# LittlePey/TASeg

Measured on AMD Instinct MI355X. Metric: scans/sec (train fwd+bwd) at ~120k pts/scan, higher is better.
Workload: dtype f32

## Files before the change

### include/taseg_hip.h

```cpp
#ifndef TASEG_HIP_H_
#define TASEG_HIP_H_

#include <stddef.h>
#include <stdint.h>

#ifdef __cplusplus
extern "C" {
#endif

#define TS_OK 0
#define TS_ERR_INVALID_ARGUMENT (-1)
#define TS_ERR_WORKSPACE_TOO_SMALL (-2)
#define TS_ERR_LAUNCH_FAILED (-3)
#define TS_ERR_UNSUPPORTED (-4)

typedef void *ts_stream_t;

const char *ts_version(void);
const char *ts_last_error(void);

enum {
  TS_OPT_GATHER_POSITIONS = 0,
  TS_OPT_WGRAD_WGS = 1,
  TS_OPT_EVAL_TAIL_SEPARATE = 2,
// ... 371 lines not shown
                      const void *labels, int32_t label_bytes, int64_t n_lab, const int64_t *num_points,
                      const int64_t *num_points_ms, int64_t *hist, int32_t *pred, int64_t pred_cap, int32_t *flags,
                      ts_stream_t stream);
int ts_eval_votes(const void *logits, int32_t half, int32_t C, int64_t n_vox, const int64_t *counts, const int32_t *scene_flags,
                  int32_t n_scenes, const int64_t *inv, const int32_t *rows, const int64_t *kept, int64_t n_pts,
                  const int64_t *num_points, const int64_t *num_points_ms, void *label, int32_t label_bytes, float *sums,
                  float *top3, int64_t cap, int64_t *n_out, int32_t *flags, ts_stream_t stream);
int ts_eval_confusion_rows(const void *logits, int32_t half, int32_t C, int64_t n_vox, const int64_t *counts,
                           const int32_t *scene_flags, int32_t n_scenes, const int64_t *grows, int64_t n_pts, const void *labels,
                           int32_t label_bytes, const int64_t *num_points, int64_t *hist, int32_t *pred, int64_t pred_cap,
                           int64_t *m_out, int32_t *flags, ts_stream_t stream);
int ts_eval_votes_rows(const void *logits, int32_t half, int32_t C, int64_t n_vox, const int64_t *counts, const int32_t *scene_flags,
                       int32_t n_scenes, const int64_t *grows, int64_t n_pts, const int64_t *num_points, void *label,
                       int32_t label_bytes, float *sums, float *top3, int64_t cap, int64_t *n_out, int32_t *flags,
                       ts_stream_t stream);
int ts_cat_cols(const void *a, int64_t a_bytes, const void *b, int64_t b_bytes, int64_t rows, void *dst, ts_stream_t stream);
int ts_copy_cols(const void *src, int64_t src_pitch, int64_t offset, int64_t width, int64_t rows, void *dst, int64_t dst_pitch,
                 ts_stream_t stream);
int ts_conv_block_forward(const void *feat, int64_t n_feat_rows, int32_t c_in, const float *kernel, int32_t K,
                          const int32_t *nbmaps, const int32_t *nboffs, int64_t n_pairs, int32_t gather_col,
                          const int32_t *pos, int64_t n_out, int32_t c_out, const void *residual, const float *bn_weight,
                          const float *bn_bias, float *running_mean, float *running_var, int64_t *num_batches_tracked,
                          float eps, float momentum, int32_t relu, int32_t half, void *comm, double *pack, void *conv_out,
                          float *mean, float *invstd, void *out, uint8_t *mask, void *w16, const TsConvBlockOpts *opts,
                          void *ws, size_t ws_bytes, ts_stream_t stream);
int ts_conv_block_eval(const void *feat, int64_t n_feat_rows, int32_t c_in, const float *kernel, int32_t K,
                       const int32_t *nbmaps, const int32_t *nboffs, int64_t n_pairs, int32_t gather_col, const int32_t *pos,
                       int64_t n_out, int32_t c_out, const void *residual, const float *bn_weight, const float *bn_bias,
                       const float *mean, const float *invstd, int32_t relu, int32_t half, void *out, void *w16,
                       const TsConvBlockOpts *opts, void *ws, size_t ws_bytes, ts_stream_t stream);
int ts_conv_block_backward(const void *grad_out, const uint8_t *mask, const void *conv_out, const float *mean,
                           const float *invstd, const float *bn_weight, const double *total_dev, void *comm, double *sums,
                           int64_t n_out, int32_t c_out, int32_t half, const void *feat, int64_t n_feat_rows, int32_t c_in,
                           const void *weights, int32_t K, const int32_t *nbmaps, const int32_t *nboffs, int64_t n_pairs,
                           int32_t dgrad_gather_col, const int32_t *pos_dgrad, int64_t n_dgrad_rows, int32_t wgrad_col_a,
                           void *grad_feat, void *grad_residual, float *grad_kernel, float *grad_bn_weight,
                           float *grad_bn_bias, const TsConvBlockOpts *opts, void *ws, size_t ws_bytes, ts_stream_t stream);

void ts_prof_enable(int32_t on);
int ts_prof_reserve(int64_t n_events);
int64_t ts_prof_collect(double *records, int64_t capacity);
int ts_prof_empty_bracket_us(int32_t reps, ts_stream_t stream, double *out_us);

void ts_set_conv_impl(int32_t impl);

int ts_lovasz_errors(const float *probas, const int64_t *labels, int64_t ignore, int64_t n_points, int32_t n_classes,
                     float *errors, ts_stream_t stream);
size_t ts_lovasz_workspace_bytes(int64_t n_points, int32_t n_classes);
int ts_lovasz_grad(const float *errors_sorted, const int64_t *perm, const int64_t *labels, int64_t ignore, int64_t n_points,
                   int32_t n_classes, float *loss, float *grad_probas, int32_t class_major, void *ws, size_t ws_bytes,
                   ts_stream_t stream);

int ts_softmax_ce_forward(const float *logits, const int64_t *labels, int64_t ignore, int64_t n_points, int32_t n_classes,
                          float *probas, float *errors, double *partials, ts_stream_t stream);
int ts_ce_lovasz_finish(const double *partials, int64_t n_points, int32_t n_classes, float smoothing, float w_ce, float w_lov,
                        const float *lovasz, float *out4, ts_stream_t stream);
int ts_ce_lovasz_backward(const float *probas, const int64_t *labels, int64_t ignore, const float *grad_probas,
                          const float *out4, const float *grad_out, int64_t n_points, int32_t n_classes, float smoothing,
                          float w_ce, float w_lov, float *grad_logits, ts_stream_t stream);

typedef struct TsPlaneJob {
  const float *w;
  void *planes;
  int32_t K, c_in, c_out;
} TsPlaneJob;
int ts_conv_split_planes(const float *w, int32_t K, int32_t c_in, int32_t c_out, void *planes, ts_stream_t stream);
int ts_conv_split_planes_batch(const TsPlaneJob *jobs, int32_t n_jobs, ts_stream_t stream);
void ts_conv_planes_hint(const float *w, const void *planes, int32_t K, int32_t c_in, int32_t c_out);
int ts_cast_weights_f16_batch(const TsPlaneJob *jobs, int32_t n_jobs, ts_stream_t stream);

int64_t ts_conv_class_rows(int64_t n);
int64_t ts_conv_class_rows2(int64_t n, int32_t groups);
size_t ts_conv_class_plan_workspace_bytes(int64_t n);
int ts_conv_class_plan(const int32_t *nbr, int64_t n, int32_t K, int32_t groups, int32_t *src, int32_t *tile_info,
                       int32_t *n_tiles, int32_t *pos, int32_t *rows, void *ws, size_t ws_bytes, ts_stream_t stream);
int ts_conv_class_plan_pairs(const int32_t *nbmaps, const int32_t *nboffs, int32_t K, int64_t n_pairs, int32_t *src,
                             int32_t *tile_info, int32_t *n_tiles, int32_t *rows, void *ws, size_t ws_bytes, ts_stream_t stream);
int ts_conv_nbr_transposed(const int32_t *pos_in, const int32_t *nbmaps, int32_t K, int64_t n_in, int32_t *nbr_t,
                           ts_stream_t stream);
int32_t ts_conv_class_supported(int32_t c_red, int32_t c_out);
int ts_conv_class_gemm(const float *feat, int32_t c_red, const float *kernel, int32_t K, int32_t groups, int32_t c_out,
                       const int32_t *src, int64_t m_pad, const int32_t *tile_info, const int32_t *n_tiles, int32_t wt,
                       int32_t mirror, const int32_t *rows, float *zp, ts_stream_t stream);
int32_t ts_conv_class_finish_pays(int64_t n, int32_t half);
int ts_conv_class_conv(const float *feat, int32_t c_red, const float *kernel, int32_t K, int32_t groups, int32_t c_out,
                       const int32_t *src, int64_t m_pad, const int32_t *tile_info, const int32_t *n_tiles, int32_t wt,
                       int32_t mirror, const int32_t *pos, int64_t n, const float *addend, float *zp, float *out,
                       ts_stream_t stream);
int ts_conv_class_gemm_f16(const void *feat, int32_t c_red, const void *w, int32_t K, int32_t groups, int32_t c_out,
                           const int32_t *src, int64_t m_pad, const int32_t *tile_info, const int32_t *n_tiles, int32_t wt,
                           int32_t mirror, const int32_t *rows, void *zp, ts_stream_t stream);
int ts_conv_class_conv_f16(const void *feat, int32_t c_red, const void *w, int32_t K, int32_t groups, int32_t c_out,
                           const int32_t *src, int64_t m_pad, const int32_t *tile_info, const int32_t *n_tiles, int32_t wt,
                           int32_t mirror, const int32_t *pos, int64_t n, const void *addend, void *zp, void *out,
                           ts_stream_t stream);

void ts_debug_phase_stamps(unsigned long long *stamps, int64_t capacity);


int ts_voxel_coords(const float *points, int64_t n, int32_t point_stride, float voxel_size,
                    const int32_t *batch_idx, int32_t n_batch, const int32_t *shift_in,
                    int32_t *mins_out, int32_t *out_coords, ts_stream_t stream);

int ts_segment_min3(const float *points, int64_t n, int32_t point_stride, const int64_t *seg, int32_t n_seg, float *out,
                    ts_stream_t stream);
int ts_stage_keep_flags(const float *points, int64_t n, int32_t point_stride, const uint8_t *pre_keep, const int32_t *scan_idx,
                        const int64_t *cls, const uint8_t *table, int32_t n_scans, int32_t table_cols, int32_t neg_col,
                        const int64_t *sample_of_scan, const float *lo, int32_t n_samples, uint8_t *keep, int64_t *sample,
                        ts_stream_t stream);
int ts_stage_layout(const float *cur, const int64_t *cur_lab, const int64_t *cur_b, int64_t n_cur, const float *hist,
                    const int64_t *hist_lab, const int64_t *hist_b, const int64_t *idx, int64_t n_kept, int32_t f,
                    const int64_t *cur_start, const int64_t *kept_start, float *pts, int64_t *lab, int64_t *sample, int32_t *sample32,
                    uint8_t *is_cur, ts_stream_t stream);
int ts_stage_split_voxels(const int32_t *coords4, const int32_t *index, int64_t m, const int32_t *inverse,
                          const int64_t *row_sample, int64_t n, int32_t n_samples, int32_t *vox, int64_t *start, int32_t *offset,
                          int64_t *inverse_local, ts_stream_t stream);
#define TS_AUG_RECORD 8
int ts_stage_augment(const float *points, int64_t n, int32_t point_stride, const int32_t *sample_idx, const double *params,
                     int32_t n_samples, float *out, ts_stream_t stream);
#define TS_MIX_RECORD 24
#define TS_MIX_MAX_CLASSES 16
size_t ts_stage_mix_workspace_bytes(int64_t n_rows, int64_t n_blocks, int32_t n_jobs);
int ts_stage_mix(const float *points, int64_t n_rows, int32_t point_stride, const int64_t *labels, const uint8_t *keep,
                 const double *records, const int32_t *classes, int32_t n_jobs, int64_t n_blocks, float *out, int64_t *out_labels,
                 int32_t *out_job, int64_t capacity, int64_t *totals, void *ws, size_t ws_bytes, ts_stream_t stream);
#define TS_CLAMP_MAX_SAMPLES 64
size_t ts_stage_clamp_compact_workspace_bytes(int64_t n, int32_t n_samples);
int ts_stage_clamp_compact(const float *points, int64_t n, int32_t point_stride, const int64_t *labels, const int32_t *sample,
                           const float *lo, int32_t n_samples, float *out, int64_t *out_labels, int64_t *out_sample,
                           int32_t *out_sample32, int64_t *counts, void *ws, size_t ws_bytes, ts_stream_t stream);
#define TS_STAGE_PAIR_MAX_SAMPLES 64
size_t ts_stage_layout_pair_workspace_bytes(int64_t n_hist, int32_t n_samples);
int ts_stage_layout_pair(const float *cur, int64_t n_cur, int32_t cur_stride, const int64_t *cur_labels, const int64_t *cur_start,
                         const float *hist, int64_t n_hist, const int64_t *hist_labels, const int32_t *scan_idx,
                         const int64_t *cls_a, const int64_t *cls_b, const uint8_t *table_a, const uint8_t *table_b,
                         int32_t n_scans, int32_t table_cols, int32_t neg_col, const int64_t *sample_of_scan, const float *lo,
                         int32_t n_samples, float *out_a, int64_t *out_labels_a, int64_t *out_sample_a, int32_t *out_sample32_a,
                         uint8_t *out_is_cur_a, float *out_b, int64_t *out_sample_b, int32_t *out_sample32_b, int64_t capacity,
                         int64_t *counts, void *ws, size_t ws_bytes, ts_stream_t stream);
#define TS_MOVING_STATS 9
#define TS_MOVING_RECORD 8
#define TS_MOVING_MAX_CANDIDATES 1024
size_t ts_stage_moving_workspace_bytes(int64_t n_rows, int32_t cap, int64_t cap_rows);
int ts_stage_moving_stats(const float *points, int64_t n_rows, int64_t n_cur, int32_t point_stride, const int64_t *labels,
                          const int32_t *cloud, const int32_t *delta, const int64_t *cand, const int32_t *cand_start,
                          int32_t n_clouds, int32_t cap, int64_t cap_rows, int32_t *counts, float *stats, int64_t *matched, void *ws,
                          size_t ws_bytes, ts_stream_t stream);
int ts_stage_moving_apply(float *points, int64_t n_rows, int64_t n_cur, int32_t point_stride, const int64_t *labels,
                          const int32_t *cloud, const int32_t *delta, const int64_t *rec_labels, const int32_t *rec_start,
                          int32_t n_clouds, const double *records, const int64_t *lut, int64_t *out_labels, ts_stream_t stream);
size_t ts_quantize_workspace_bytes(int64_t n);
int ts_sparse_quantize(const int32_t *coords, int64_t n, int32_t *out_index, int32_t *out_inverse,
                       int32_t *out_count, void *ws, size_t ws_bytes, ts_stream_t stream);
#define TS_CYL_FLAG_WORDS 3
#define TS_CYL_FLAG_NONFINITE 1
#define TS_CYL_FLAG_LABEL 2
#define TS_CYL_FLAG_RANGE 4
int ts_cylinder_cells(const float *points, int64_t n, int32_t point_stride, const int32_t *sample_idx, const double *space,
                      int32_t *cells, int64_t *point_coord, float *point_feature, int32_t *flags, ts_stream_t stream);
size_t ts_cylinder_voxels_workspace_bytes(int64_t n, int32_t n_samples);
int ts_cylinder_voxels(const int32_t *cells, const int64_t *labels, int64_t n, int32_t n_samples, int32_t num_classes,
                       int64_t ignore_label, int32_t *out_index, int64_t *out_inverse, int64_t *voxel_label, int32_t *counts,
                       int32_t *flags, void *ws, size_t ws_bytes, ts_stream_t stream);

int ts_fuse_scan(const float *points, int64_t n, const float *pose0, const float *pose,
                 float *out, ts_stream_t stream);
// ... 62 lines not shown
```

### taseg_amd/_lib.py

```python
import ctypes
import os
import threading

import torch

_HERE = os.path.dirname(os.path.abspath(__file__))
from .options import options as _options

LIB_PATH = _options.hip_lib or os.path.join(_HERE, "libtaseg_hip.so")

TS_OK = 0
_c = ctypes
_vp, _i64, _i32, _sz = _c.c_void_p, _c.c_int64, _c.c_int32, _c.c_size_t

SIGNATURES = {
    "ts_version": (_c.c_char_p, []),
    "ts_last_error": (_c.c_char_p, []),
    "ts_set_option": (_i32, [_i32, _i64]),
    "ts_get_option": (_i64, [_i32]),
    "ts_hash": (_i32, [_vp, _i64, _vp, _vp]),
    "ts_kernel_hash": (_i32, [_vp, _i64, _vp, _i32, _vp, _vp]),
    "ts_hash_query_workspace_bytes": (_sz, [_i64]),
    "ts_hash_query": (_i32, [_vp, _i64, _vp, _vp, _i64, _vp, _vp, _sz, _vp]),
    "ts_count": (_i32, [_vp, _i64, _vp, _i64, _vp]),
# ... 80 lines not shown
    "ts_conv3x3_rows_pack": (_i32, [_vp, _i32, _i32, _i64, _i64, _i64, _i64, _i32, _vp, _vp]),
    "ts_conv3x3_rows": (_i32, [_vp, _i32, _vp, _vp, _i32, _i32, _i32, _vp, _i32, _vp]),
    "ts_conv1x1c32_packed_bytes": (_sz, []),
    "ts_conv1x1c32_pack": (_i32, [_vp, _i64, _i64, _i32, _vp, _vp]),
    "ts_conv1x1c32_rows": (_i32, [_vp, _vp, _vp, _i64, _i32, _c.c_float, _vp, _vp]),
    "ts_conv1x1c32_wgrad": (_i32, [_vp, _vp, _i32, _i32, _i32, _vp, _i64, _i64, _vp, _vp, _sz, _vp]),
    "ts_conv3x3_wgrad_workspace_bytes": (_sz, [_i32, _i32]),
    "ts_conv3x3_wgrad": (_i32, [_vp, _i32, _vp, _i32, _i32, _i32, _i32, _vp, _i64, _i64, _i64, _i64, _vp, _vp, _sz, _vp]),
    "ts_conv3x3c32_wgrad_workspace_bytes": (_sz, []),
    "ts_conv3x3c32_wgrad": (_i32, [_vp, _vp, _i32, _i32, _i32, _i32, _vp, _i64, _i64, _i64, _i64, _vp, _vp, _sz, _vp]),
    "ts_cast_weights_f16": (_i32, [_vp, _i32, _i32, _i32, _vp, _vp, _vp]),
    "ts_conv_pair_gemm_f16": (_i32, [_vp, _i64, _i32, _vp, _i32, _vp, _vp, _i64, _i32, _vp, _i32, _vp]),
    "ts_conv_pair_gemm_f16_nat": (_i32, [_vp, _i64, _i32, _vp, _i32, _vp, _vp, _i64, _i32, _vp, _i32, _vp]),
    "ts_conv_gather_sum_f16": (_i32, [_vp, _i32, _vp, _i32, _i64, _i64, _vp, _vp]),
    "ts_conv_wgrad_f16": (_i32, [_vp, _i32, _vp, _i32, _vp, _vp, _i32, _i32, _i64, _vp, _vp]),
    "ts_bn_act_train_forward_f16": (_i32, [_vp, _vp, _vp, _vp, _vp, _vp, _vp, _i64, _i32, _c.c_float, _c.c_float, _i32,
                                           _vp, _vp, _vp, _vp, _vp, _sz, _vp]),
    "ts_bn_act_train_backward_f16": (_i32, [_vp, _vp, _vp, _vp, _vp, _vp, _i64, _i32, _vp, _vp, _vp, _vp, _vp, _sz, _vp]),
    "ts_sgd_grad_stats": (_i32, [_vp, _i64, _vp, _vp, _vp]),
    "ts_sgd_decide": (_i32, [_vp, _vp, _vp, _c.c_float, _c.c_float, _c.c_float, _i32, _i32, _vp]),
    "ts_sgd_apply": (_i32, [_vp, _vp, _vp, _i64, _vp, _c.c_float, _c.c_float, _c.c_float, _i32, _vp]),
    "ts_sgd_apply_segments": (_i32, [_vp, _vp, _vp, _i64, _vp, _vp, _i32, _vp, _i64, _vp, _vp, _i32, _c.c_float, _c.c_float,
                                     _c.c_float, _i32, _i32, _vp]),
    "ts_bn_sync_stats_f16": (_i32, [_vp, _i64, _i32, _vp, _vp, _sz, _vp]),
    "ts_bn_act_forward_f16": (_i32, [_vp, _vp, _vp, _vp, _vp, _vp, _i64, _i32, _i32, _vp, _vp, _vp]),
    "ts_bn_sync_backward_reduce_f16": (_i32, [_vp, _vp, _vp, _vp, _vp, _i64, _i32, _vp, _vp, _vp, _vp, _sz, _vp]),
    "ts_bn_act_backward_f16": (_i32, [_vp, _vp, _vp, _vp, _vp, _vp, _vp, _vp, _c.c_double, _i64, _i32, _vp, _vp, _vp, _sz,
                                      _vp]),
    "ts_rccl_load": (_i32, [_c.c_char_p]),
    "ts_rccl_unique_id": (_i32, [_vp]),
    "ts_rccl_comm_init": (_i32, [_vp, _i32, _i32, _c.POINTER(_vp)]),
    "ts_rccl_comm_destroy": (_i32, [_vp]),
    "ts_rccl_allreduce_f64": (_i32, [_vp, _vp, _i64, _vp]),
    "ts_bn_sync_forward": (_i32, [_vp, _vp, _vp, _vp, _vp, _vp, _vp, _vp, _i64, _i32, _c.c_float, _c.c_float, _i32, _i32, _vp,
                                  _vp, _vp, _vp, _vp, _vp, _sz, _vp]),
    "ts_bn_sync_backward": (_i32, [_vp, _vp, _vp, _vp, _vp, _vp, _vp, _vp, _i64, _i32, _i32, _vp, _vp, _vp, _vp, _vp, _vp,
                                   _sz, _vp]),
    "ts_conv_block_workspace_bytes": (_sz, [_i64, _i64, _i32, _i32, _i32, _i32]),
    "ts_conv_block_wgrad_ws_bytes": (_sz, [_i64, _i64, _i32, _i32, _i32, _i32]),
    "ts_stream_join": (_i32, [_vp, _vp]),
    "ts_conv_block_wgrad_side": (_i32, [_vp, _i64, _i32, _i32, _vp, _vp, _i64, _i32, _i64, _i32, _i32, _vp, _i32, _vp, _sz, _i32, _vp]),
    "ts_set_device": (_i32, [_i32]),
    "ts_scene_counts": (_i32, [_vp, _i64, _i64, _vp, _i64, _i64, _vp, _i64, _i64, _i32, _vp, _vp, _vp]),
    "ts_unvoxelise": (_i32, [_vp, _i32, _i32, _vp, _i32, _vp, _i64, _vp, _i64, _vp, _vp, _vp, _vp]),
    "ts_eval_rows_workspace_bytes": (_sz, [_i64, _i32]),
    "ts_eval_rows": (_i32, [_vp, _vp, _i64, _vp, _i64, _i32, _vp, _vp, _vp, _sz, _vp]),
    "ts_eval_confusion": (_i32, [_vp, _i32, _i32, _i64, _vp, _vp, _i32, _vp, _vp, _vp, _i64, _vp, _i32, _i64, _vp, _vp, _vp, _vp, _i64,
                                 _vp, _vp]),
    "ts_eval_votes": (_i32, [_vp, _i32, _i32, _i64, _vp, _vp, _i32, _vp, _vp, _vp, _i64, _vp, _vp, _vp, _i32, _vp, _vp, _i64, _vp, _vp,
                             _vp]),
    "ts_eval_confusion_rows": (_i32, [_vp, _i32, _i32, _i64, _vp, _vp, _i32, _vp, _i64, _vp, _i32, _vp, _vp, _vp, _i64, _vp, _vp, _vp]),
    "ts_eval_votes_rows": (_i32, [_vp, _i32, _i32, _i64, _vp, _vp, _i32, _vp, _i64, _vp, _vp, _i32, _vp, _vp, _i64, _vp, _vp, _vp]),
    "ts_cat_cols": (_i32, [_vp, _i64, _vp, _i64, _i64, _vp, _vp]),
    "ts_copy_cols": (_i32, [_vp, _i64, _i64, _i64, _i64, _vp, _i64, _vp]),
    "ts_conv_block_forward": (_i32, [_vp, _i64, _i32, _vp, _i32, _vp, _vp, _i64, _i32, _vp, _i64, _i32, _vp, _vp, _vp, _vp,
                                     _vp, _vp, _c.c_float, _c.c_float, _i32, _i32, _vp, _vp, _vp, _vp, _vp, _vp, _vp, _vp,
                                     _vp, _vp, _sz, _vp]),
    "ts_conv_block_eval": (_i32, [_vp, _i64, _i32, _vp, _i32, _vp, _vp, _i64, _i32, _vp, _i64, _i32, _vp, _vp, _vp, _vp, _vp, _i32,
                                  _i32, _vp, _vp, _vp, _vp, _sz, _vp]),
    "ts_conv_block_backward": (_i32, [_vp, _vp, _vp, _vp, _vp, _vp, _vp, _vp, _vp, _i64, _i32, _i32, _vp, _i64, _i32, _vp,
                                      _i32, _vp, _vp, _i64, _i32, _vp, _i64, _i32, _vp, _vp, _vp, _vp, _vp, _vp, _vp, _sz,
                                      _vp]),
    "ts_prof_enable": (None, [_i32]),
    "ts_prof_reserve": (_i32, [_i64]),
    "ts_prof_collect": (_i64, [_vp, _i64]),
    "ts_prof_empty_bracket_us": (_i32, [_i32, _vp, _vp]),
    "ts_set_conv_impl": (None, [_i32]),
    "ts_softmax_ce_forward": (_i32, [_vp, _vp, _i64, _i64, _i32, _vp, _vp, _vp, _vp]),
    "ts_ce_lovasz_finish": (_i32, [_vp, _i64, _i32, _c.c_float, _c.c_float, _c.c_float, _vp, _vp, _vp]),
    "ts_ce_lovasz_backward": (_i32, [_vp, _vp, _i64, _vp, _vp, _vp, _i64, _i32, _c.c_float, _c.c_float, _c.c_float, _vp, _vp]),
    "ts_lovasz_errors": (_i32, [_vp, _vp, _i64, _i64, _i32, _vp, _vp]),
    "ts_lovasz_workspace_bytes": (_sz, [_i64, _i32]),
    "ts_lovasz_grad": (_i32, [_vp, _vp, _vp, _i64, _i64, _i32, _vp, _vp, _i32, _vp, _sz, _vp]),
    "ts_conv_split_planes": (_i32, [_vp, _i32, _i32, _i32, _vp, _vp]),
    "ts_conv_split_planes_batch": (_i32, [_vp, _i32, _vp]),
    "ts_cast_weights_f16_batch": (_i32, [_vp, _i32, _vp]),
    "ts_conv_class_rows": (_i64, [_i64]),
    "ts_conv_class_rows2": (_i64, [_i64, _i32]),
    "ts_conv_class_plan_workspace_bytes": (_sz, [_i64]),
    "ts_conv_class_plan": (_i32, [_vp, _i64, _i32, _i32, _vp, _vp, _vp, _vp, _vp, _vp, _sz, _vp]),
    "ts_conv_class_plan_pairs": (_i32, [_vp, _vp, _i32, _i64, _vp, _vp, _vp, _vp, _vp, _sz, _vp]),
    "ts_conv_nbr_transposed": (_i32, [_vp, _vp, _i32, _i64, _vp, _vp]),
    "ts_conv_class_supported": (_i32, [_i32, _i32]),
    "ts_conv_class_gemm": (_i32, [_vp, _i32, _vp, _i32, _i32, _i32, _vp, _i64, _vp, _vp, _i32, _i32, _vp, _vp, _vp]),
    "ts_conv_class_gemm_f16": (_i32, [_vp, _i32, _vp, _i32, _i32, _i32, _vp, _i64, _vp, _vp, _i32, _i32, _vp, _vp, _vp]),
    "ts_conv_class_finish_pays": (_i32, [_i64, _i32]),
    "ts_conv_class_conv": (_i32, [_vp, _i32, _vp, _i32, _i32, _i32, _vp, _i64, _vp, _vp, _i32, _i32, _vp, _i64, _vp, _vp, _vp, _vp]),
    "ts_conv_class_conv_f16": (_i32, [_vp, _i32, _vp, _i32, _i32, _i32, _vp, _i64, _vp, _vp, _i32, _i32, _vp, _i64, _vp, _vp, _vp, _vp]),
    "ts_conv_planes_hint": (None, [_vp, _vp, _i32, _i32, _i32]),
    "ts_debug_phase_stamps": (None, [_vp, _i64]),
    "ts_fuse_scan": (_i32, [_vp, _i64, _vp, _vp, _vp, _vp]),
    "ts_fuse_scans": (_i32, [_vp, _vp, _i64, _vp, _vp, _i32, _vp, _vp]),
    "ts_fuse_scans_batch": (_i32, [_vp, _vp, _i64, _vp, _vp, _i32, _vp, _vp]),
    "ts_fuse_sweeps": (_i32, [_vp, _vp, _i64, _vp, _i32, _vp, _vp, _vp]),
    "ts_project_fov": (_i32, [_vp, _i64, _vp, _i32, _i32, _i32, _i32, _c.c_float, _vp, _vp, _vp]),
    "ts_project_cam": (_i32, [_vp, _i64, _vp, _i32, _i32, _i32, _c.c_float, _vp, _vp, _vp]),
    "ts_tiaf_image_stack": (_i32, [_vp, _vp, _vp, _vp, _vp, _i32, _vp, _i32, _i32, _i64, _i64, _vp, _vp, _vp]),
    "ts_tiaf_fov_cloud_workspace_bytes": (_sz, [_i64, _i32]),
    "ts_tiaf_fov_cloud": (_i32, [_vp, _i64, _vp, _i64, _vp, _i32, _vp, _vp, _i32, _i32, _i32, _vp, _vp, _vp, _i64, _vp, _vp, _sz, _vp]),
    "ts_nusc_fov_cloud_workspace_bytes": (_sz, [_i64, _i32]),
    "ts_nusc_fov_cloud": (_i32, [_vp, _vp, _vp, _i64, _vp, _i64, _vp, _i32, _vp, _vp, _i32, _vp, _vp, _vp, _vp, _i64, _vp, _vp, _sz, _vp]),
    "ts_segment_min3": (_i32, [_vp, _i64, _i32, _vp, _i32, _vp, _vp]),
    "ts_stage_keep_flags": (_i32, [_vp, _i64, _i32, _vp, _vp, _vp, _vp, _i32, _i32, _i32, _vp, _vp, _i32, _vp, _vp, _vp]),
    "ts_stage_augment": (_i32, [_vp, _i64, _i32, _vp, _vp, _i32, _vp, _vp]),
    "ts_stage_mix_workspace_bytes": (_sz, [_i64, _i64, _i32]),
    "ts_stage_mix": (_i32, [_vp, _i64, _i32, _vp, _vp, _vp, _vp, _i32, _i64, _vp, _vp, _vp, _i64, _vp, _vp, _sz, _vp]),
    "ts_stage_clamp_compact_workspace_bytes": (_sz, [_i64, _i32]),
    "ts_stage_clamp_compact": (_i32, [_vp, _i64, _i32, _vp, _vp, _vp, _i32, _vp, _vp, _vp, _vp, _vp, _vp, _sz, _vp]),
    "ts_stage_layout_pair_workspace_bytes": (_sz, [_i64, _i32]),
    "ts_stage_layout_pair": (_i32, [_vp, _i64, _i32, _vp, _vp, _vp, _i64, _vp, _vp, _vp, _vp, _vp, _vp, _i32, _i32, _i32, _vp, _vp,
                                    _i32, _vp, _vp, _vp, _vp, _vp, _vp, _vp, _vp, _i64, _vp, _vp, _sz, _vp]),
    "ts_stage_moving_workspace_bytes": (_sz, [_i64, _i32, _i64]),
    "ts_stage_moving_stats": (_i32, [_vp, _i64, _i64, _i32, _vp, _vp, _vp, _vp, _vp, _i32, _i32, _i64, _vp, _vp, _vp, _vp, _sz, _vp]),
    "ts_stage_moving_apply": (_i32, [_vp, _i64, _i64, _i32, _vp, _vp, _vp, _vp, _vp, _i32, _vp, _vp, _vp, _vp]),
    "ts_stage_layout": (_i32, [_vp, _vp, _vp, _i64, _vp, _vp, _vp, _vp, _i64, _i32, _vp, _vp, _vp, _vp, _vp, _vp, _vp, _vp]),
    "ts_stage_split_voxels": (_i32, [_vp, _vp, _i64, _vp, _vp, _i64, _i32, _vp, _vp, _vp, _vp, _vp]),
    "ts_quantize_workspace_bytes": (_sz, [_i64]),
    "ts_sparse_quantize": (_i32, [_vp, _i64, _vp, _vp, _vp, _vp, _sz, _vp]),
    "ts_voxel_coords": (_i32, [_vp, _i64, _i32, _c.c_float, _vp, _i32, _vp, _vp, _vp, _vp]),
    "ts_cylinder_cells": (_i32, [_vp, _i64, _i32, _vp, _c.POINTER(_c.c_double), _vp, _vp, _vp, _vp, _vp]),
    "ts_cylinder_voxels_workspace_bytes": (_sz, [_i64, _i32]),
    "ts_cylinder_voxels": (_i32, [_vp, _vp, _i64, _i32, _i32, _i64, _vp, _vp, _vp, _vp, _vp, _vp, _sz, _vp]),
}



SGD_TILE = 4096


class TsClassPlan(_c.Structure):
    _fields_ = [("src", _vp), ("tile_info", _vp), ("n_tiles", _vp), ("pos", _vp), ("rows", _vp), ("n", _i64), ("m_pad", _i64),
                ("z_rows", _i64), ("K", _i32), ("groups", _i32), ("mirror", _i32), ("map_id", _vp)]


class TsConvBlockOpts(_c.Structure):
    _fields_ = [("fwd_plan", _c.POINTER(TsClassPlan)), ("dgrad_plan", _c.POINTER(TsClassPlan)), ("planes", _vp),
                ("w16_current", _i32), ("addend", _vp), ("wgrad_stream", _vp), ("wgrad_ws", _vp), ("wgrad_ws_bytes", _sz),
                ("wgrad_slot", _i32), ("wgrad_deferred", _i32), ("natural", _i32)]


_lib = None
_lock = threading.Lock()


class BackendError(RuntimeError):
    """A libtaseg_hip entry point returned a TS_ERR_* code."""


def load():
    global _lib
    if _lib is not None:
        return _lib
    with _lock:
        if _lib is None:
            if not os.path.exists(LIB_PATH):
                raise ImportError(
                    f"{LIB_PATH} is missing: build it with `python -m taseg_amd.csrc.build` "
                    "(or __graft_entry__.build()).  taseg_amd has no CPU fallback.")
            lib = ctypes.CDLL(LIB_PATH)
            for name, (res, args) in SIGNATURES.items():
                fn = getattr(lib, name)
                fn.restype = res
                fn.argtypes = args
            push_options(lib)
            _lib = lib
    return _lib
# ... 55 lines not shown
```

### taseg_amd/backend.py

```python
import torch

from . import _lib as L
from ._lib import BackendError, check
from .options import options

__all__ = [
    "hash_cuda", "kernel_hash_cuda", "hash_query_cuda", "count_cuda",
    "voxelize_forward_cuda", "voxelize_backward_cuda",
    "devoxelize_forward_cuda", "devoxelize_backward_cuda", "devox_order", "devoxelize_backward_runs", "devox_csr",
    "devoxelize_backward_csr",
    "convolution_forward_cuda", "convolution_backward_cuda",
    "downsample", "unique_i64", "build_kmap", "trilinear_map", "conv_nbr", "conv_wgrad", "conv_class_plan", "conv_class_gemm", "conv_class_gemm_f16", "conv_class_conv", "conv_class_conv_f16", "class_finish_pays",
    "fuse_scan", "fuse_scans", "fuse_sweeps", "project_fov", "voxel_coords", "sparse_quantize", "set_conv_impl", "image_gather_forward", "image_gather_backward", "image_gather_rows_forward", "image_gather_rows_backward", "avgpool3s2_rows_forward", "avgpool3s2_rows_backward", "conv3x3c32_pack", "conv3x3c32_rows", "conv3x3c32_wgrad", "conv3x3_rows_takes", "conv3x3_rows_pack", "conv3x3_rows", "conv3x3_wgrad", "conv1x1c32_pack", "conv1x1c32_rows", "conv1x1c32_wgrad", "shuffle_cat_rows_takes", "shuffle_cat_rows_forward", "shuffle_cat_rows_backward",
    "eval_confusion", "eval_votes", "eval_confusion_rows", "eval_votes_rows",
    "voxelize_max_forward", "voxelize_max_backward", "sigmoid3_gate_forward", "sigmoid3_gate_backward",
    "point_groups", "voxelize_mean_piece_rows", "voxelize_mean_forward", "voxelize_mean_backward", "point_tail_forward",
]


def _f32(t, name):
    if t.dtype != torch.float32:
        raise TypeError(f"{name} must be float32 (got {t.dtype}); the HIP path computes in f32")
    return t.contiguous()

# ... 894 lines not shown
            raise ValueError("conv3x3_rows: bias length")
    y = torch.empty((t, int(out_channels), h, w), dtype=x.dtype, device=x.device, memory_format=torch.channels_last)
    L.check(lib.ts_conv3x3_rows(L.ptr(x), c, L.ptr(packed), L.ptr(bias), t, h, w, L.ptr(y), int(out_channels), L.stream()),
            "ts_conv3x3_rows")
    return y


def conv1x1c32_pack(weight, mode):
    L.require_device(weight)
    if weight.dtype != torch.float16 or tuple(weight.shape) != (32, 32, 1, 1):
        raise ValueError(f"conv1x1c32_pack: a float16 [32, 32, 1, 1] weight, got {weight.dtype} {tuple(weight.shape)}")
    lib = L.load()
    packed = torch.empty(lib.ts_conv1x1c32_packed_bytes(), dtype=torch.uint8, device=weight.device)
    L.check(lib.ts_conv1x1c32_pack(L.ptr(weight), weight.stride(0), weight.stride(1), int(mode), L.ptr(packed), L.stream()), "ts_conv1x1c32_pack")
    return packed


def conv1x1c32_rows(x, packed, bias, slope=None):
    L.require_device(x, packed, bias)
    x = _channels_last_rows(x, "conv1x1c32_rows")
    t, c, h, w = x.shape
    if c != 32 or x.dtype != torch.float16:
        raise ValueError(f"conv1x1c32_rows: float16 with 32 channels, got {x.dtype} with {c}")
    if bias is not None:
        bias = _f32(bias, "bias")
    y = torch.empty_like(x, memory_format=torch.channels_last)
    L.check(L.load().ts_conv1x1c32_rows(L.ptr(x), L.ptr(packed), L.ptr(bias), t * h * w, int(slope is not None), float(slope or 0.0), L.ptr(y),
                                        L.stream()), "ts_conv1x1c32_rows")
    return y


def conv1x1c32_wgrad(x, g, like_weight):
    L.require_device(x, g)
    x, g = _channels_last_rows(x, "conv1x1c32_wgrad(x)"), _channels_last_rows(g, "conv1x1c32_wgrad(g)")
    if x.shape != g.shape or x.shape[1] != 32 or x.dtype != torch.float16 or g.dtype != torch.float16 or tuple(like_weight.shape) != (32, 32, 1, 1):
        raise ValueError("conv1x1c32_wgrad: two float16 [T, 32, H, W] stacks of one shape and a [32, 32, 1, 1] weight")
    t, _, h, w = x.shape
    gw = torch.empty_like(like_weight, dtype=torch.float16)
    gb = torch.empty(32, dtype=torch.float32, device=x.device)
    lib = L.load()
    ws = L.workspace(lib.ts_conv3x3c32_wgrad_workspace_bytes(), x.device)
    L.check(lib.ts_conv1x1c32_wgrad(L.ptr(x), L.ptr(g), t, h, w, L.ptr(gw), gw.stride(0), gw.stride(1), L.ptr(gb), L.ptr(ws), ws.numel(), L.stream()),
            "ts_conv1x1c32_wgrad")
    return gw, gb


def conv3x3_wgrad(x, grad_y, like_weight, want_bias=True):
    L.require_device(x, grad_y)
    x, grad_y = _channels_last_rows(x, "conv3x3_wgrad(x)"), _channels_last_rows(grad_y, "conv3x3_wgrad(grad_y)")
    t, ci, h, w = x.shape
    co = grad_y.shape[1]
    lib = L.load()
    need = lib.ts_conv3x3_wgrad_workspace_bytes(ci, co)
    if (x.dtype != torch.float16 or grad_y.dtype != torch.float16 or tuple(grad_y.shape) != (t, co, h, w) or need == 0
            or tuple(like_weight.shape) != (co, ci, 3, 3)):
        raise ValueError(f"conv3x3_wgrad: float16 stacks {tuple(x.shape)} / {tuple(grad_y.shape)} and a weight like {tuple(like_weight.shape)}")
    gw = torch.empty_like(like_weight, dtype=torch.float16)
    gb = torch.empty(co, dtype=torch.float32, device=x.device) if want_bias else None
    s = gw.stride()
    ws = L.workspace(need, x.device)
    L.check(lib.ts_conv3x3_wgrad(L.ptr(x), ci, L.ptr(grad_y), co, t, h, w, L.ptr(gw), s[0], s[1], s[2], s[3], L.ptr(gb), L.ptr(ws), ws.numel(),
                                 L.stream()), "ts_conv3x3_wgrad")
    return gw, gb


def conv3x3c32_wgrad(x, grad_y, like_weight, dilation, want_bias=False):
    L.require_device(x, grad_y)
    x, grad_y = _channels_last_rows(x, "conv3x3c32_wgrad(x)"), _channels_last_rows(grad_y, "conv3x3c32_wgrad(grad_y)")
    if x.shape != grad_y.shape or x.shape[1] != 32 or x.dtype != torch.float16 or grad_y.dtype != torch.float16:
        raise ValueError("conv3x3c32_wgrad: two float16 [T, 32, H, W] stacks of one shape")
    t, _, h, w = x.shape
    gw = torch.empty_like(like_weight, dtype=torch.float16)
    gb = torch.empty(32, dtype=torch.float32, device=x.device) if want_bias else None
    s = gw.stride()
    lib = L.load()
    ws = L.workspace(lib.ts_conv3x3c32_wgrad_workspace_bytes(), x.device)
    L.check(lib.ts_conv3x3c32_wgrad(L.ptr(x), L.ptr(grad_y), t, h, w, int(dilation), L.ptr(gw), s[0], s[1], s[2], s[3], L.ptr(gb), L.ptr(ws),
                                    ws.numel(), L.stream()), "ts_conv3x3c32_wgrad")
    return (gw, gb) if want_bias else gw


def set_conv_impl(impl):
    global _conv_impl
    _conv_impl = int(impl)
    L.load().ts_set_conv_impl(int(impl))


def fuse_scan(points, pose0, pose):
    L.require_device(points, pose0, pose)
    points, pose0, pose = _f32(points, "points"), _f32(pose0, "pose0"), _f32(pose, "pose")
    assert points.ndim == 2 and points.shape[1] == 4 and pose0.shape == (4, 4) and pose.shape == (4, 4)
    out = torch.empty_like(points)
    L.check(L.load().ts_fuse_scan(L.ptr(points), points.shape[0], L.ptr(pose0), L.ptr(pose), L.ptr(out), L.stream()),
            "ts_fuse_scan")
    return out


def fuse_scans(points, scan_idx, pose0, poses):
    L.require_device(points, scan_idx, pose0, poses)
    points, pose0, poses = _f32(points, "points"), _f32(pose0, "pose0"), _f32(poses, "poses")
    scan_idx = _i32(scan_idx, "scan_idx")
    assert points.ndim == 2 and points.shape[1] == 4 and pose0.shape == (4, 4) and poses.shape[1:] == (4, 4)
    out = torch.empty_like(points)
    L.check(L.load().ts_fuse_scans(L.ptr(points), L.ptr(scan_idx), points.shape[0], L.ptr(pose0), L.ptr(poses),
                                   poses.shape[0], L.ptr(out), L.stream()), "ts_fuse_scans")
    return out


def fuse_scans_batch(points, scan_idx, pose0s, poses):
    L.require_device(points, scan_idx, pose0s, poses)
    points, pose0s, poses = _f32(points, "points"), _f32(pose0s, "pose0s"), _f32(poses, "poses")
    scan_idx = _i32(scan_idx, "scan_idx")
    assert points.ndim == 2 and points.shape[1] == 4 and pose0s.shape == poses.shape and poses.shape[1:] == (4, 4)
    out = torch.empty_like(points)
    if points.shape[0]:
        L.check(L.load().ts_fuse_scans_batch(L.ptr(points), L.ptr(scan_idx), points.shape[0], L.ptr(pose0s), L.ptr(poses),
                                             poses.shape[0], L.ptr(out), L.stream()), "ts_fuse_scans_batch")
    return out


def fuse_sweeps(points, sweep_idx, params):
    L.require_device(points, sweep_idx, params)
    points, sweep_idx = _f32(points, "points"), _i32(sweep_idx, "sweep_idx")
    if params.dtype != torch.float64 or params.ndim != 2 or params.shape[1] != 28:
        raise TypeError("params must be float64 [S, 28]")
    params = params.contiguous()
    assert points.ndim == 2 and points.shape[1] == 5, points.shape
    out = torch.empty_like(points)
    keep = torch.empty(points.shape[0], dtype=torch.uint8, device=points.device)
    L.check(L.load().ts_fuse_sweeps(L.ptr(points), L.ptr(sweep_idx), points.shape[0], L.ptr(params), params.shape[0],
                                    L.ptr(out), L.ptr(keep), L.stream()), "ts_fuse_sweeps")
    return out, keep.bool()


def project_fov(points, proj, image_size, crop, row_offset=0.0):
    L.require_device(points, proj)
    points = _f32(points, "points")
    if proj.dtype != torch.float64 or tuple(proj.shape) != (3, 4):
        raise TypeError("proj must be float64 [3, 4]")
    proj = proj.contiguous()
    assert points.ndim == 2 and points.shape[1] == 4, points.shape
    n = points.shape[0]
    pix = torch.empty((n, 2), dtype=torch.float32, device=points.device)
    keep = torch.empty(n, dtype=torch.uint8, device=points.device)
    L.check(L.load().ts_project_fov(L.ptr(points), n, L.ptr(proj), int(image_size[0]), int(image_size[1]), int(crop[0]),
                                    int(crop[1]), float(row_offset), L.ptr(pix), L.ptr(keep), L.stream()), "ts_project_fov")
    return pix, keep.bool()


def project_cam(points, cam, image_size, crop_top, row_offset=0.0):
    L.require_device(points, cam)
    points = _f32(points, "points")
    if cam.dtype != torch.float64 or cam.numel() != 57:
        raise TypeError("cam must be 57 float64 values")
    cam = cam.contiguous()
    assert points.ndim == 2 and points.shape[1] == 4, points.shape
    n = points.shape[0]
    pix = torch.empty((n, 2), dtype=torch.float32, device=points.device)
    keep = torch.empty(n, dtype=torch.uint8, device=points.device)
    L.check(L.load().ts_project_cam(L.ptr(points), n, L.ptr(cam), int(image_size[0]), int(image_size[1]), int(crop_top),
                                    float(row_offset), L.ptr(pix), L.ptr(keep), L.stream()), "ts_project_cam")
    return pix, keep.bool()


def voxel_coords(points, voxel_size, batch_idx=None, n_batch=1, shift=None):
    L.require_device(points, batch_idx, shift)
    points = _f32(points, "points")
# ... 421 lines not shown
    dev = cells.device
    if counts is None:
        counts = torch.empty(nb + 1, dtype=torch.int32, device=dev)
    if flags is None:
        flags = torch.zeros(CYL_FLAG_WORDS, dtype=torch.int32, device=dev)
    for t, size, name in ((counts, nb + 1, "counts"), (flags, CYL_FLAG_WORDS, "flags")):
        if t.dtype != torch.int32 or t.shape != (size,) or not t.is_contiguous():
            raise TypeError("%s must be a contiguous int32 [%d] tensor" % (name, size))
    lib = L.load()
    ws = L.workspace(lib.ts_cylinder_voxels_workspace_bytes(n, nb), dev)
    index = torch.empty(max(n, 1), dtype=torch.int32, device=dev)
    inverse = torch.empty(max(n, 1), dtype=torch.int64, device=dev)
    voxel_label = torch.empty(max(n, 1), dtype=torch.int64, device=dev)
    L.check(lib.ts_cylinder_voxels(L.ptr(cells), L.ptr(labels), n, nb, int(num_classes), int(ignore_label), L.ptr(index),
                                   L.ptr(inverse), L.ptr(voxel_label), L.ptr(counts), L.ptr(flags), L.ptr(ws), ws.numel(),
                                   L.stream()), "ts_cylinder_voxels")
    return index, inverse[:n], voxel_label, counts, flags


def _tile_cols(c):
    return 128 if c % 128 == 0 else 96 if c % 96 == 0 else 64 if c % 64 == 0 else 32


def conv_class_plan(nbr, groups=3, direct=False):
    L.require_device(nbr)
    nbr = _i32(nbr, "nbr")
    k, n = nbr.shape
    if direct:
        groups = 1
    lib = L.load()
    m_pad = int(lib.ts_conv_class_rows2(n, groups))
    dev = nbr.device
    src = torch.empty((k // groups, m_pad), dtype=torch.int32, device=dev)
    tile_info = torch.empty((max(m_pad // 128, 1), 2), dtype=torch.int32, device=dev)
    n_tiles = torch.empty(2, dtype=torch.int32, device=dev)
    pos = None if direct else torch.empty((groups, n), dtype=torch.int32, device=dev)
    rows = torch.empty(m_pad, dtype=torch.int32, device=dev) if direct else None
    ws = L.workspace(lib.ts_conv_class_plan_workspace_bytes(n), dev)
    L.check(lib.ts_conv_class_plan(L.ptr(nbr), n, k, groups, L.ptr(src), L.ptr(tile_info), L.ptr(n_tiles), L.ptr(pos), L.ptr(rows),
                                   L.ptr(ws), ws.numel(), L.stream()), "ts_conv_class_plan")
    return dict(src=src, tile_info=tile_info, n_tiles=n_tiles, pos=pos, rows=rows, m_pad=m_pad, n=n, K=k, groups=groups,
                mirror=0 if direct else 1, z_rows=0, map_id=None)


def conv_class_plan_pairs(nbmaps, nboffs, k, n_pairs):
    L.require_device(nbmaps, nboffs)
    nbmaps, nboffs = _i32(nbmaps, "nbmaps"), _i32(nboffs, "nboffs")
    lib = L.load()
    n = int(n_pairs)
    m_pad = int(lib.ts_conv_class_rows2(n, 1))
    dev = nbmaps.device
    src = torch.empty((k, m_pad), dtype=torch.int32, device=dev)
    tile_info = torch.empty((max(m_pad // 128, 1), 2), dtype=torch.int32, device=dev)
    n_tiles = torch.empty(2, dtype=torch.int32, device=dev)
    rows = torch.empty(m_pad, dtype=torch.int32, device=dev)
    ws = L.workspace(4 * (m_pad // 128) + 256, dev)
    L.check(lib.ts_conv_class_plan_pairs(L.ptr(nbmaps), L.ptr(nboffs), k, n, L.ptr(src), L.ptr(tile_info), L.ptr(n_tiles),
                                         L.ptr(rows), L.ptr(ws), ws.numel(), L.stream()), "ts_conv_class_plan_pairs")
    return dict(src=src, tile_info=tile_info, n_tiles=n_tiles, pos=None, rows=rows, m_pad=m_pad, n=n, K=k, groups=1, mirror=0,
                z_rows=0, map_id=None)


def conv_nbr_transposed(pos_in, nbmaps, k):
    L.require_device(pos_in, nbmaps)
    pos_in, nbmaps = _i32(pos_in, "pos_in"), _i32(nbmaps, "nbmaps")
    n_in = pos_in.shape[1]
    out = torch.empty((k, n_in), dtype=torch.int32, device=pos_in.device)
    L.check(L.load().ts_conv_nbr_transposed(L.ptr(pos_in), L.ptr(nbmaps), k, n_in, L.ptr(out), L.stream()),
            "ts_conv_nbr_transposed")
    return out


def class_plan_struct(plan):
    st = plan.get("_struct")
    if st is None:
        mid = plan.get("map_id")
        st = L.TsClassPlan(L.ptr(plan["src"]), L.ptr(plan["tile_info"]), L.ptr(plan["n_tiles"]), L.ptr(plan["pos"]),
                           L.ptr(plan["rows"]), plan["n"], plan["m_pad"], int(plan.get("z_rows") or 0), plan["K"], plan["groups"],
                           plan["mirror"], None if mid is None else mid.data_ptr())
        plan["_struct"] = st
    return st


def conv_class_gemm(feat, kernel, plan, weight_transposed=False):
    L.require_device(feat, kernel)
    feat, kernel = _f32(feat, "feat"), _f32(kernel, "kernel")
    k, c_in, c_out = kernel.shape
    c_red, cols = (c_out, c_in) if weight_transposed else (c_in, c_out)
    if feat.shape[1] != c_red:
        raise ValueError(f"conv_class_gemm: feat has {feat.shape[1]} channels, the product reduces over {c_red}")
    direct = plan["rows"] is not None
    zp = torch.empty((plan["n"] if direct else plan["m_pad"], cols), dtype=torch.float32, device=feat.device)
    with _Timed("class_gemm", name=f"class_gemm_kernel<{_tile_cols(cols)}>", pairs=int(plan.get("pairs", 0)), c_red=c_red,
                c_out=cols, k=k, esize=4, n_rows=feat.shape[0], z_rows=0 if direct else int(plan.get("z_rows") or plan["m_pad"]),
                out_rows=plan["n"] if direct else 0):
        L.check(L.load().ts_conv_class_gemm(L.ptr(feat), c_red, L.ptr(kernel), k, plan["groups"], cols, L.ptr(plan["src"]),
                                            plan["m_pad"], L.ptr(plan["tile_info"]), L.ptr(plan["n_tiles"]),
                                            1 if weight_transposed else 0, plan["mirror"], L.ptr(plan["rows"]), L.ptr(zp),
                                            L.stream()), "ts_conv_class_gemm")
    return zp


def _z_moves(plan):
    z = int(plan.get("z_rows") or plan["m_pad"])
    return 2 * max(0, z - (plan["n"] + 127) // 128 * 128)


def class_finish_pays(n, half=False):
    return bool(L.load().ts_conv_class_finish_pays(int(n), 1 if half else 0))


def conv_class_conv(feat, kernel, plan, weight_transposed=False, addend=None):
    L.require_device(feat, kernel)
    feat, kernel = _f32(feat, "feat"), _f32(kernel, "kernel")
    k, c_in, c_out = kernel.shape
    c_red, cols = (c_out, c_in) if weight_transposed else (c_in, c_out)
    if feat.shape[1] != c_red:
        raise ValueError(f"conv_class_conv: feat has {feat.shape[1]} channels, the product reduces over {c_red}")
    if plan["rows"] is not None or plan["groups"] != 3:
        raise ValueError("conv_class_conv: a three-group pass-2 plan is needed")
    if addend is not None:
        addend = _f32(addend, "addend")
        if addend.shape != (plan["n"], cols):
            raise ValueError(f"conv_class_conv: addend shape {tuple(addend.shape)} != {(plan['n'], cols)}")
    zp = torch.empty((plan["m_pad"], cols), dtype=torch.float32, device=feat.device)
    out = torch.empty((plan["n"], cols), dtype=torch.float32, device=feat.device)
    with _Timed("class_gemm", name=f"class_gemm_kernel<{_tile_cols(cols)}>", pairs=int(plan.get("pairs", 0)), c_red=c_red,
                c_out=cols, k=k, esize=4, n_rows=feat.shape[0], z_rows=_z_moves(plan), out_rows=plan["n"]):
        L.check(L.load().ts_conv_class_conv(L.ptr(feat), c_red, L.ptr(kernel), k, 3, cols, L.ptr(plan["src"]), plan["m_pad"],
                                            L.ptr(plan["tile_info"]), L.ptr(plan["n_tiles"]), 1 if weight_transposed else 0,
                                            plan["mirror"], L.ptr(plan["pos"]), plan["n"], L.ptr(addend), L.ptr(zp), L.ptr(out),
                                            L.stream()), "ts_conv_class_conv")
    return out


def conv_class_conv_f16(feat, w16, plan, weight_transposed=False, addend=None):
    L.require_device(feat, w16)
    if feat.dtype != torch.float16 or w16.dtype != torch.float16 or (addend is not None and addend.dtype != torch.float16):
        raise TypeError("conv_class_conv_f16: half tensors expected")
    feat, w16 = feat.contiguous(), w16.contiguous()
    k, c_in, c_out = w16.shape
    c_red, cols = (c_out, c_in) if weight_transposed else (c_in, c_out)
    if feat.shape[1] != c_red:
        raise ValueError(f"conv_class_conv_f16: feat has {feat.shape[1]} channels, the product reduces over {c_red}")
    if plan["rows"] is not None or plan["groups"] != 3:
        raise ValueError("conv_class_conv_f16: a three-group pass-2 plan is needed")
    if addend is not None:
        addend = addend.contiguous()
        if addend.shape != (plan["n"], cols):
            raise ValueError(f"conv_class_conv_f16: addend shape {tuple(addend.shape)} != {(plan['n'], cols)}")
    zp = torch.empty((plan["m_pad"], cols), dtype=torch.float16, device=feat.device)
    out = torch.empty((plan["n"], cols), dtype=torch.float16, device=feat.device)
    with _Timed("class_gemm", name=f"class_gemm_kernel<{_tile_cols(cols)}>", pairs=int(plan.get("pairs", 0)), c_red=c_red,
                c_out=cols, k=k, esize=2, n_rows=feat.shape[0], z_rows=_z_moves(plan), out_rows=plan["n"]):
        L.check(L.load().ts_conv_class_conv_f16(L.ptr(feat), c_red, L.ptr(w16), k, 3, cols, L.ptr(plan["src"]), plan["m_pad"],
                                                L.ptr(plan["tile_info"]), L.ptr(plan["n_tiles"]), 1 if weight_transposed else 0,
                                                plan["mirror"], L.ptr(plan["pos"]), plan["n"], L.ptr(addend), L.ptr(zp),
                                                L.ptr(out), L.stream()), "ts_conv_class_conv_f16")
    return out


def conv_class_gemm_f16(feat, w16, plan, weight_transposed=False):
    L.require_device(feat, w16)
    if feat.dtype != torch.float16 or w16.dtype != torch.float16:
        raise TypeError("conv_class_gemm_f16: half tensors expected")
    feat, w16 = feat.contiguous(), w16.contiguous()
    k, c_in, c_out = w16.shape
    c_red, cols = (c_out, c_in) if weight_transposed else (c_in, c_out)
    if feat.shape[1] != c_red:
        raise ValueError(f"conv_class_gemm_f16: feat has {feat.shape[1]} channels, the product reduces over {c_red}")
    direct = plan["rows"] is not None
    zp = torch.empty((plan["n"] if direct else plan["m_pad"], cols), dtype=torch.float16, device=feat.device)
    with _Timed("class_gemm", name=f"class_gemm_kernel<{_tile_cols(cols)}>", pairs=int(plan.get("pairs", 0)), c_red=c_red,
                c_out=cols, k=k, esize=2, n_rows=feat.shape[0], z_rows=0 if direct else int(plan.get("z_rows") or plan["m_pad"]),
                out_rows=plan["n"] if direct else 0):
        L.check(L.load().ts_conv_class_gemm_f16(L.ptr(feat), c_red, L.ptr(w16), k, plan["groups"], cols, L.ptr(plan["src"]),
                                                plan["m_pad"], L.ptr(plan["tile_info"]), L.ptr(plan["n_tiles"]),
                                                1 if weight_transposed else 0, plan["mirror"], L.ptr(plan["rows"]), L.ptr(zp),
# ... 317 lines not shown
```

### taseg_amd/csrc/block.hip

```cpp
#include <sched.h>

#include <atomic>
#include <mutex>
#include <vector>

#include "common.h"

static inline size_t blk_align(size_t x) { return ts_align_up(x, 256); }

extern "C" size_t ts_conv_block_workspace_bytes(int64_t n_pairs, int64_t n_rows_max, int32_t c_in, int32_t c_out,
                                                int32_t K, int32_t half) {
  const size_t es = half ? 2 : 4;
  const size_t cmax = (size_t)std::max(c_in, c_out);
  size_t total = blk_align((size_t)n_pairs * cmax * es);
  total += blk_align((size_t)n_rows_max * cmax * es);
  if (half) total += blk_align((size_t)K * c_in * c_out * 2);
  total += blk_align(ts_bn_train_workspace_bytes(std::max(c_in, c_out)));
  total += blk_align(ts_wgrad_partial_bytes(n_pairs, c_in, c_out, K));
  return total;
}

extern "C" size_t ts_conv_block_wgrad_ws_bytes(int64_t n_pairs, int64_t n_out, int32_t c_in, int32_t c_out, int32_t K, int32_t half) {
  const size_t es = half ? 2 : 4;
  return blk_align((size_t)n_out * (size_t)std::max(c_in, c_out) * es) + blk_align(ts_wgrad_partial_bytes(n_pairs, c_in, c_out, K));
// ... 131 lines not shown
  for (auto &e : ev) TS_CHECK_HIP(hipEventRecord(e, stream), "hipEventRecord");
  TS_CHECK_HIP(hipEventSynchronize(ev.back()), "hipEventSynchronize");
  std::vector<double> us;
  for (int i = 0; i < reps; ++i) {
    float ms = 0.f;
    TS_CHECK_HIP(hipEventElapsedTime(&ms, ev[2 * i], ev[2 * i + 1]), "hipEventElapsedTime");
    us.push_back(1e3 * ms);
  }
  std::sort(us.begin(), us.end());
  *out_us = us[us.size() / 2];
  for (auto &e : ev) g_prof_pool.push_back(e);
  return TS_OK;
}

struct PlanesScope {
  TsPlanesHint h;
  PlanesScope(const float *w, const void *planes, int K, int c_in, int c_out)
      : h{planes ? w : nullptr, (const unsigned short *)planes, K, c_in, c_out} {
    g_ts_planes_hint = TsPlanesHint{nullptr, nullptr, 0, 0, 0};
  }
  void arm() const { g_ts_planes_hint = h; }
  ~PlanesScope() { g_ts_planes_hint = TsPlanesHint{nullptr, nullptr, 0, 0, 0}; }
};

static bool plan_fits(const TsClassPlan *p, int32_t K, int64_t n_dest, int32_t c_red, int32_t c_out, int64_t n_pairs,
                      const int32_t *nboffs) {
  if (!p || !p->src || !p->tile_info || !p->n_tiles || g_ts_conv_impl != 0) return false;
  if (p->K != K || p->n != n_dest || p->map_id != (const void *)nboffs || !ts_conv_class_supported(c_red, c_out)) return false;
  if (p->groups < 1 || K % p->groups != 0 || p->m_pad != ts_conv_class_rows2(n_dest, p->groups)) return false;
  if (p->rows) return p->groups == 1 && !p->pos;
  return p->pos && p->m_pad <= n_pairs;
}
static double plan_z_rows(const TsClassPlan *p) { return (double)(p->z_rows > 0 ? p->z_rows : p->m_pad); }
static bool plan_finishes(const TsClassPlan *p, int32_t half) {
  return p && !p->rows && p->pos && p->groups == 3 && p->K == 27 && ts_conv_class_finish_pays(p->n, half);
}
static double plan_z_moves(const TsClassPlan *p, int64_t n) {
  return 2.0 * std::max(0.0, plan_z_rows(p) - (double)((n + 127) / 128 * 128));
}

static int block_conv(const void *feat, int64_t n_feat_rows, int32_t c_in, const float *kernel, int32_t K, const int32_t *nbmaps,
                      const int32_t *nboffs, int64_t n_pairs, int32_t gather_col, const int32_t *pos, int64_t n_out, int32_t c_out,
                      int32_t half, void *conv_out, void *w16, const TsConvBlockOpts &o, const PlanesScope &planes, void *z,
                      ts_stream_t stream, const TsGatherEpilogue *tail = nullptr, void *tail_out = nullptr, bool *tail_done = nullptr) {
  auto pass2 = [&](const void *zz, const int32_t *table, int32_t kk, int64_t zrows) -> int {
    if (tail && tail_out) {
      const int rc = half ? ts_conv_gather_sum_f16_epi(zz, c_out, table, kk, n_out, zrows, tail_out, *tail, stream)
                          : ts_conv_gather_sum_epi((const float *)zz, c_out, table, kk, n_out, zrows, (float *)tail_out, *tail, stream);
      if (rc == TS_OK) {
        if (tail_done) *tail_done = true;
        return TS_OK;
      }
      if (rc != TS_ERR_UNSUPPORTED) return rc;
    }
    return half ? ts_conv_gather_sum_f16(zz, c_out, table, kk, n_out, zrows, conv_out, stream)
                : ts_conv_gather_sum((const float *)zz, c_out, table, kk, n_out, zrows, (float *)conv_out, stream);
  };
  if (o.natural) {
    TS_REQUIRE(K == 1 && n_pairs == n_out && n_feat_rows == n_out, TS_ERR_INVALID_ARGUMENT,
               "ts_conv_block: a natural call needs K = 1 and one pair per row (%d offsets, %lld pairs, %lld / %lld rows)", K,
               (long long)n_pairs, (long long)n_feat_rows, (long long)n_out);
    if (half && !o.w16_current) TS_TRY(ts_cast_weights_f16(kernel, K, c_in, c_out, w16, nullptr, stream));
    ProfScope ps(0, stream, (double)n_pairs, c_in, c_out, K, (double)n_feat_rows, half ? 2 : 4, 0);
    if (half) return ts_conv_pair_gemm_f16_nat(feat, n_feat_rows, c_in, w16, K, nbmaps, nboffs, n_pairs, gather_col, conv_out, c_out, stream);
    return ts_conv_pair_gemm((const float *)feat, n_feat_rows, c_in, kernel, K, 0, nbmaps, nboffs, n_pairs, gather_col,
                             (float *)conv_out, c_out, stream);
  }
  const TsClassPlan *cp = plan_fits(o.fwd_plan, K, n_out, c_in, c_out, n_pairs, nboffs) ? o.fwd_plan : nullptr;
  {
    if (half && !o.w16_current) TS_TRY(ts_cast_weights_f16(kernel, K, c_in, c_out, w16, nullptr, stream));
    const double es_d = half ? 2 : 4;
    if (cp) {
      const bool fused = plan_finishes(cp, half);
      void *dst = cp->rows ? conv_out : z;
      const TsClassFinish fin = {cp->pos, n_out, conv_out, nullptr};
      {
        ProfScope ps(fused ? 4 : 3, stream, (double)n_pairs, c_in, c_out, K, (double)n_feat_rows, es_d,
                     cp->rows ? -(double)n_out : fused ? plan_z_moves(cp, n_out) : plan_z_rows(cp));
        if (half)
          TS_TRY(ts_conv_class_gemm_f16_ex(feat, c_in, w16, K, cp->groups, c_out, cp->src, cp->m_pad, cp->tile_info, cp->n_tiles,
                                           0, 0, cp->rows, dst, nullptr, fused ? &fin : nullptr, stream));
        else
          TS_TRY(ts_conv_class_gemm_ex((const float *)feat, c_in, kernel, K, cp->groups, c_out, cp->src, cp->m_pad, cp->tile_info,
                                       cp->n_tiles, 0, 0, cp->rows, (float *)dst, nullptr, fused ? &fin : nullptr, stream));
      }
      if (!cp->rows && !fused) {
        ProfScope ps(1, stream, plan_z_rows(cp), 0, c_out, cp->groups, (double)n_out, es_d, 0);
        TS_TRY(pass2(z, cp->pos, cp->groups, cp->m_pad));
      }
    } else if (half) {
      {
        ProfScope ps(0, stream, (double)n_pairs, c_in, c_out, K, (double)n_feat_rows, 2, 0);
        TS_TRY(ts_conv_pair_gemm_f16_nat(feat, n_feat_rows, c_in, w16, K, nbmaps, nboffs, n_pairs, gather_col, z, c_out, stream));
      }
      {
        ProfScope ps(1, stream, (double)n_pairs, 0, c_out, K, (double)n_out, 2, 0);
        TS_TRY(pass2(z, pos, K, n_pairs));
      }
    } else {
      {
        ProfScope ps(0, stream, (double)n_pairs, c_in, c_out, K, (double)n_feat_rows, 4, 0);
        planes.arm();
        TS_TRY(ts_conv_pair_gemm((const float *)feat, n_feat_rows, c_in, kernel, K, 0, nbmaps, nboffs, n_pairs, gather_col,
                                 (float *)z, c_out, stream));
      }
      {
        ProfScope ps(1, stream, (double)n_pairs, 0, c_out, K, (double)n_out, 4, 0);
        TS_TRY(pass2(z, pos, K, n_pairs));
      }
    }
  }
  return TS_OK;
}

extern "C" int ts_conv_block_forward(const void *feat, int64_t n_feat_rows, int32_t c_in, const float *kernel, int32_t K,
                                     const int32_t *nbmaps, const int32_t *nboffs, int64_t n_pairs, int32_t gather_col,
                                     const int32_t *pos, int64_t n_out, int32_t c_out, const void *residual,
                                     const float *bn_weight, const float *bn_bias, float *running_mean,
                                     float *running_var, int64_t *num_batches_tracked, float eps, float momentum,
                                     int32_t relu, int32_t half, void *comm, double *pack, void *conv_out, float *mean,
                                     float *invstd, void *out, uint8_t *mask, void *w16, const TsConvBlockOpts *opts, void *ws,
                                     size_t ws_bytes, ts_stream_t stream) {
  const TsConvBlockOpts none = {};
  const TsConvBlockOpts &o = opts ? *opts : none;
  PlanesScope planes(kernel, half ? nullptr : o.planes, K, c_in, c_out);
  TS_REQUIRE(n_pairs > 0 && n_out > 0 && c_in > 0 && c_out > 0 && K > 0, TS_ERR_INVALID_ARGUMENT,
             "ts_conv_block_forward: bad sizes");
  TS_REQUIRE(ws && ws_bytes >= ts_conv_block_workspace_bytes(n_pairs, n_out, c_in, c_out, K, half), TS_ERR_INVALID_ARGUMENT,
             "ts_conv_block_forward: workspace too small");
  TS_REQUIRE(!half || w16, TS_ERR_INVALID_ARGUMENT, "ts_conv_block_forward: half storage needs the w16 buffer");
  const size_t es = half ? 2 : 4;
  const size_t cmax = (size_t)std::max(c_in, c_out);
  char *p = (char *)ws;
  void *z = p;
  p += blk_align((size_t)n_pairs * cmax * es);
  p += blk_align((size_t)n_out * cmax * es);
  if (half) p += blk_align((size_t)K * c_in * c_out * 2);
  void *bn_ws = p;
  const size_t bn_ws_bytes = ts_bn_train_workspace_bytes(std::max(c_in, c_out));
  if (comm == TS_COMM_CALLER_POST) {
  } else {
    TS_TRY(block_conv(feat, n_feat_rows, c_in, kernel, K, nbmaps, nboffs, n_pairs, gather_col, pos, n_out, c_out, half, conv_out,
                      w16, o, planes, z, stream));
  }
  if (comm)
    return ts_bn_sync_forward(comm, conv_out, residual, bn_weight, bn_bias, running_mean, running_var, num_batches_tracked,
                              n_out, c_out, eps, momentum, relu, half, pack, mean, invstd, out, mask, bn_ws, bn_ws_bytes,
                              stream);
  if (half)
    return ts_bn_act_train_forward_f16(conv_out, residual, bn_weight, bn_bias, running_mean, running_var,
                                       num_batches_tracked, n_out, c_out, eps, momentum, relu, mean, invstd, out, mask,
                                       bn_ws, bn_ws_bytes, stream);
  return ts_bn_act_train_forward((const float *)conv_out, (const float *)residual, bn_weight, bn_bias, running_mean,
                                 running_var, num_batches_tracked, n_out, c_out, eps, momentum, relu, mean, invstd,
                                 (float *)out, mask, bn_ws, bn_ws_bytes, stream);
}

extern "C" int ts_conv_block_eval(const void *feat, int64_t n_feat_rows, int32_t c_in, const float *kernel, int32_t K,
                                  const int32_t *nbmaps, const int32_t *nboffs, int64_t n_pairs, int32_t gather_col,
                                  const int32_t *pos, int64_t n_out, int32_t c_out, const void *residual, const float *bn_weight,
                                  const float *bn_bias, const float *mean, const float *invstd, int32_t relu, int32_t half,
                                  void *out, void *w16, const TsConvBlockOpts *opts, void *ws, size_t ws_bytes,
                                  ts_stream_t stream) {
  const TsConvBlockOpts none = {};
  const TsConvBlockOpts &o = opts ? *opts : none;
  PlanesScope planes(kernel, half ? nullptr : o.planes, K, c_in, c_out);
  TS_REQUIRE(n_pairs > 0 && n_out > 0 && c_in > 0 && c_out > 0 && K > 0, TS_ERR_INVALID_ARGUMENT, "ts_conv_block_eval: bad sizes");
// ... 66 lines not shown
               TS_ERR_INVALID_ARGUMENT, "ts_conv_block_backward: weight-gradient ring slot / scratch");
    TS_TRY(wg_events());
    grad_conv = o.wgrad_ws;
    side_part = (float *)((char *)o.wgrad_ws + blk_align((size_t)n_out * cmax * es));
    for (int spin = 0; g_wg_owed[o.wgrad_slot].load(std::memory_order_acquire) != 0; ++spin) {
      if (spin > 64) sched_yield();
      if (spin > 20000000) {
        g_wg_owed[o.wgrad_slot].store(0, std::memory_order_release);
        break;
      }
    }
    if (g_wg_used[o.wgrad_slot].load() && hipEventQuery(g_wg_done[o.wgrad_slot]) != hipSuccess) {
      (void)hipGetLastError();
      TS_CHECK_HIP(hipStreamWaitEvent((hipStream_t)stream, g_wg_done[o.wgrad_slot], 0), "ring wait");
    }
  }
  if (comm) {
    TS_TRY(ts_bn_sync_backward(comm, grad_out, mask, conv_out, mean, invstd, bn_weight, total_dev, n_out, c_out, half, sums,
                               grad_conv, grad_residual, grad_bn_weight, grad_bn_bias, bn_ws, bn_ws_bytes, stream));
  } else if (half) {
    TS_TRY(ts_bn_act_train_backward_f16(grad_out, mask, conv_out, mean, invstd, bn_weight, n_out, c_out, grad_conv,
                                        grad_residual, grad_bn_weight, grad_bn_bias, bn_ws, bn_ws_bytes, stream));
  } else {
    TS_TRY(ts_bn_act_train_backward((const float *)grad_out, mask, (const float *)conv_out, mean, invstd, bn_weight, n_out,
                                    c_out, (float *)grad_conv, (float *)grad_residual, grad_bn_weight, grad_bn_bias, bn_ws,
                                    bn_ws_bytes, stream));
  }
  const double es_d = half ? 2 : 4;
  float *part = side_on ? side_part : (float *)(((char *)bn_ws) + blk_align(bn_ws_bytes));
  const bool det = det_ok;
  TsWgradReduce job = {};
  const ts_stream_t main_stream = stream;
  const bool deferred = side_on && o.wgrad_deferred;
  if (side_on) {
    TS_CHECK_HIP(hipEventRecord(g_wg_ready[o.wgrad_slot], (hipStream_t)main_stream), "ring record");
    if (deferred) {
      g_wg_owed[o.wgrad_slot].store(1, std::memory_order_release);
    } else {
      TS_CHECK_HIP(hipStreamWaitEvent((hipStream_t)o.wgrad_stream, g_wg_ready[o.wgrad_slot], 0), "ring wait");
      stream = o.wgrad_stream;
    }
  }
  if (grad_kernel && !deferred) {
    ProfScope ps(2, stream, (double)n_pairs, c_in, c_out, K, (double)n_feat_rows, es_d, (double)n_out);
    if (det) g_ts_wgrad_part = part;
    int rc;
    if (half)
      rc = ts_conv_wgrad_f16_ex(feat, c_in, grad_conv, c_out, nbmaps, nboffs, K, wgrad_col_a, n_pairs, grad_kernel,
                                det ? 1 : 0, stream);
    else
      rc = ts_conv_wgrad_ex((const float *)feat, c_in, (const float *)grad_conv, c_out, nbmaps, nboffs, K, wgrad_col_a,
                            n_pairs, grad_kernel, det ? 1 : 0, stream);
    g_ts_wgrad_part = nullptr;
    if (rc != TS_OK) return rc;
    if (det) job = TsWgradReduce{part, nboffs, grad_kernel, K, g_ts_wgrad_plan.chunk, (int64_t)c_in * c_out / 4};
  }
  if (side_on && !deferred) {
    TS_TRY((grad_feat && n_dgrad_rows > 0 && !o.natural) ? ts_wgrad_reduce_seq(job, stream) : ts_wgrad_reduce(job, stream));
    TS_CHECK_HIP(hipEventRecord(g_wg_done[o.wgrad_slot], (hipStream_t)stream), "ring record");
    g_wg_used[o.wgrad_slot].store(true);
    stream = main_stream;
  }
  const bool ride = det && grad_feat && n_dgrad_rows > 0 && !side_on && !o.natural;
  const TsClassPlan *cp = (grad_feat && !o.natural && plan_fits(o.dgrad_plan, K, n_dgrad_rows, c_out, c_in, n_pairs, nboffs) &&
                           !(o.dgrad_plan->rows && addend))
                              ? o.dgrad_plan
                              : nullptr;
  const double side_bytes = (ride ? 4.0 * c_in * c_out * ((double)g_ts_wgrad_plan.slots + K) : 0.0) +
                            (addend ? es_d * (double)n_dgrad_rows * c_in : 0.0);
  if (cp) {
    const bool fused = plan_finishes(cp, half);
    void *dst = cp->rows ? grad_feat : z;
    const TsClassFinish fin = {cp->pos, n_dgrad_rows, grad_feat, addend};
    {
      ProfScope ps(fused ? 4 : 3, stream, (double)n_pairs, c_out, c_in, K, (double)n_out, es_d,
                   cp->rows ? -(double)n_dgrad_rows : fused ? plan_z_moves(cp, n_dgrad_rows) : plan_z_rows(cp));
      const TsWgradReduce *side = ((cp->rows || fused) && ride) ? &job : nullptr;
      if (half)
        TS_TRY(ts_conv_class_gemm_f16_ex(grad_conv, c_out, weights, K, cp->groups, c_in, cp->src, cp->m_pad, cp->tile_info,
                                         cp->n_tiles, 1, cp->mirror, cp->rows, dst, side, fused ? &fin : nullptr, stream));
      else
        TS_TRY(ts_conv_class_gemm_ex((const float *)grad_conv, c_out, (const float *)weights, K, cp->groups, c_in, cp->src,
                                     cp->m_pad, cp->tile_info, cp->n_tiles, 1, cp->mirror, cp->rows, (float *)dst, side,
                                     fused ? &fin : nullptr, stream));
    }
    if (!cp->rows && !fused) {
      ProfScope ps(1, stream, plan_z_rows(cp), 0, c_in, cp->groups, (double)n_dgrad_rows, es_d, side_bytes);
      if (half)
        TS_TRY(ts_conv_gather_sum_f16_ex(z, c_in, cp->pos, cp->groups, n_dgrad_rows, cp->m_pad, grad_feat, ride ? &job : nullptr,
                                         addend, stream));
      else
        TS_TRY(ts_conv_gather_sum_ex((const float *)z, c_in, cp->pos, cp->groups, n_dgrad_rows, cp->m_pad, (float *)grad_feat,
                                     ride ? &job : nullptr, (const float *)addend, stream));
    }
  } else if (grad_feat && o.natural) {
    ProfScope ps(0, stream, (double)n_pairs, c_out, c_in, K, (double)n_out, es_d, 1);
    if (half)
      TS_TRY(ts_conv_pair_gemm_f16(grad_conv, n_out, c_out, weights, K, nbmaps, nboffs, n_pairs, dgrad_gather_col, grad_feat, c_in,
                                   stream));
    else
      TS_TRY(ts_conv_pair_gemm((const float *)grad_conv, n_out, c_out, (const float *)weights, K, 1, nbmaps, nboffs, n_pairs,
                               dgrad_gather_col, (float *)grad_feat, c_in, stream));
  } else if (grad_feat) {
    {
      ProfScope ps(0, stream, (double)n_pairs, c_out, c_in, K, (double)n_out, es_d, 1);
      if (half)
        TS_TRY(ts_conv_pair_gemm_f16(grad_conv, n_out, c_out, weights, K, nbmaps, nboffs, n_pairs, dgrad_gather_col, z, c_in,
                                     stream));
      else {
        planes.arm();
        TS_TRY(ts_conv_pair_gemm((const float *)grad_conv, n_out, c_out, (const float *)weights, K, 1, nbmaps, nboffs,
                                 n_pairs, dgrad_gather_col, (float *)z, c_in, stream));
      }
    }
    {
      ProfScope ps(1, stream, (double)n_pairs, 0, c_in, K, (double)n_dgrad_rows, es_d, side_bytes);
      if (half)
        TS_TRY(ts_conv_gather_sum_f16_ex(z, c_in, pos_dgrad, K, n_dgrad_rows, n_pairs, grad_feat, ride ? &job : nullptr,
                                         addend, stream));
      else
        TS_TRY(ts_conv_gather_sum_ex((const float *)z, c_in, pos_dgrad, K, n_dgrad_rows, n_pairs, (float *)grad_feat,
                                     ride ? &job : nullptr, (const float *)addend, stream));
    }
  }
  if (det && !ride && !side_on) TS_TRY(ts_wgrad_reduce(job, stream));
  return TS_OK;
}

extern "C" int ts_conv_block_wgrad_side(const void *feat, int64_t n_feat_rows, int32_t c_in, int32_t K, const int32_t *nbmaps,
                                        const int32_t *nboffs, int64_t n_pairs, int32_t wgrad_col_a, int64_t n_out, int32_t c_out,
                                        int32_t half, float *grad_kernel, int32_t chunk_order, void *wgrad_ws, size_t wgrad_ws_bytes,
                                        int32_t slot, ts_stream_t side_stream) {
  TS_REQUIRE(slot >= 0 && slot < 8 && wgrad_ws && grad_kernel && feat && side_stream &&
                 wgrad_ws_bytes >= ts_conv_block_wgrad_ws_bytes(n_pairs, n_out, c_in, c_out, K, half),
             TS_ERR_INVALID_ARGUMENT, "ts_conv_block_wgrad_side: bad arguments");
  const size_t es = half ? 2 : 4;
  const size_t cmax = (size_t)std::max(c_in, c_out);
  const void *grad_conv = wgrad_ws;
  float *part = (float *)((char *)wgrad_ws + blk_align((size_t)n_out * cmax * es));
  int rc = TS_OK;
  {
    TS_CHECK_HIP(hipStreamWaitEvent((hipStream_t)side_stream, g_wg_ready[slot], 0), "ring wait");
    ProfScope ps(2, side_stream, (double)n_pairs, c_in, c_out, K, (double)n_feat_rows, half ? 2.0 : 4.0, (double)n_out);
    g_ts_wgrad_part = part;
    if (half)
      rc = ts_conv_wgrad_f16_ex(feat, c_in, grad_conv, c_out, nbmaps, nboffs, K, wgrad_col_a, n_pairs, grad_kernel, 1, side_stream);
    else
      rc = ts_conv_wgrad_ex((const float *)feat, c_in, (const float *)grad_conv, c_out, nbmaps, nboffs, K, wgrad_col_a, n_pairs,
                            grad_kernel, 1, side_stream);
    g_ts_wgrad_part = nullptr;
  }
  if (rc == TS_OK) {
    const TsWgradReduce job = {part, nboffs, grad_kernel, K, g_ts_wgrad_plan.chunk, (int64_t)c_in * c_out / 4};
    ProfScope ps(5, side_stream, 0, c_in, c_out, K, chunk_order ? 1.0 : 0.0, 4, 4.0 * c_in * c_out * ((double)g_ts_wgrad_plan.slots + K));
    rc = chunk_order ? ts_wgrad_reduce_seq(job, side_stream) : ts_wgrad_reduce(job, side_stream);
  }
  if (hipEventRecord(g_wg_done[slot], (hipStream_t)side_stream) != hipSuccess && rc == TS_OK) rc = TS_ERR_LAUNCH_FAILED;
  g_wg_used[slot].store(true);
  g_wg_owed[slot].store(0, std::memory_order_release);
  return rc;
}

extern "C" int ts_set_device(int32_t device) {
  TS_CHECK_HIP(hipSetDevice(device), "ts_set_device");
  return TS_OK;
}

// ... 62 lines not shown
```

### taseg_amd/csrc/common.h

```cpp
#pragma once
#include <hip/hip_runtime.h>
#include <stdint.h>
#include <stdio.h>

#include <algorithm>

#include "../../include/taseg_hip.h"

#define TS_WAVE 64

void ts_set_error(const char *fmt, ...);
extern int g_ts_conv_impl;

#define TS_REQUIRE(cond, code, ...)  \
  do {                               \
    if (!(cond)) {                   \
      ts_set_error(__VA_ARGS__);     \
      return (code);                 \
    }                                \
  } while (0)

#define TS_CHECK_LAUNCH(what)                                            \
  do {                                                                   \
    hipError_t e_ = hipGetLastError();                                   \
    if (e_ != hipSuccess) {                                              \
      ts_set_error("%s: launch failed: %s", what, hipGetErrorString(e_)); \
      return TS_ERR_LAUNCH_FAILED;                                       \
    }                                                                    \
  } while (0)

#define TS_CHECK_HIP(expr, what)                                      \
  do {                                                                \
    hipError_t e_ = (expr);                                           \
    if (e_ != hipSuccess) {                                           \
      ts_set_error("%s: %s", what, hipGetErrorString(e_));            \
      return TS_ERR_LAUNCH_FAILED;                                    \
    }                                                                 \
  } while (0)

static inline size_t ts_align_up(size_t x, size_t a) { return (x + a - 1) / a * a; }

static inline int64_t ts_cdiv(int64_t a, int64_t b) { return (a + b - 1) / b; }

__device__ __forceinline__ uint64_t ts_fnv60(int x, int y, int z, int b) {
  uint64_t h = 14695981039346656037ULL;
  h ^= (uint32_t)x;
  h *= 1099511628211ULL;
  h ^= (uint32_t)y;
  h *= 1099511628211ULL;
  h ^= (uint32_t)z;
  h *= 1099511628211ULL;
  h ^= (uint32_t)b;
  h *= 1099511628211ULL;
  return (h >> 60) ^ (h & 0x0FFFFFFFFFFFFFFFULL);
}

#define TS_EMPTY_KEY 0xFFFFFFFFFFFFFFFFULL

struct TsTable {
  unsigned long long *keys;
  int *vals;
  uint32_t mask;
};

static inline uint32_t ts_table_capacity(int64_t n) {
  uint64_t cap = 1024;
  while (cap < (uint64_t)(2 * n + 2)) cap <<= 1;
  return (uint32_t)cap;
}
static inline size_t ts_table_bytes(int64_t n) {
  size_t cap = ts_table_capacity(n);
  return ts_align_up(cap * 8, 256) + ts_align_up(cap * 4, 256);
}

__device__ __forceinline__ uint32_t ts_slot0(uint64_t h, uint32_t mask) {
  uint64_t m = h * 0x9E3779B97F4A7C15ULL;
  return (uint32_t)(m >> 32) & mask;
}

__device__ __forceinline__ void ts_table_insert(const TsTable &t, uint64_t key, int val) {
  uint32_t s = ts_slot0(key, t.mask);
  for (uint32_t probe = 0; probe <= t.mask; ++probe) {
    unsigned long long prev = atomicCAS(&t.keys[s], (unsigned long long)TS_EMPTY_KEY,
                                        (unsigned long long)key);
    if (prev == TS_EMPTY_KEY || prev == key) {
      atomicMin(&t.vals[s], val);
      return;
    }
    s = (s + 1) & t.mask;
  }
}

__device__ __forceinline__ int ts_table_find(const TsTable &t, uint64_t key) {
  uint32_t s = ts_slot0(key, t.mask);
  for (uint32_t probe = 0; probe <= t.mask; ++probe) {
// ... 37 lines not shown
  void *p;
  size_t bytes;
  uint32_t word;
};
int ts_fill_segments(const TsFillSeg *segs, int n, hipStream_t stream);

int ts_table_init(TsTable *t, int64_t n, void *ws, size_t ws_bytes, hipStream_t stream, size_t *used,
                  const TsFillSeg *extra = nullptr, int n_extra = 0);

size_t ts_group_slots_workspace_bytes(int64_t n_slots);
int ts_group_slots(const int32_t *idx, const float *weight, int64_t n_slots, int64_t n_vox, int32_t *offsets, int32_t *entries,
                   void *ws, size_t ws_bytes, hipStream_t stream, const char *who);

struct TsWgradPlan {
  int chunk;
  int n_chunks;
  int64_t slots;
};
static inline int ts_wgrad_wgs() {
  const int64_t v = ts_get_option(TS_OPT_WGRAD_WGS);
  return v ? (int)v : 512;
}
static inline TsWgradPlan ts_wgrad_plan(int64_t n_pairs, int tiles, int K, int step, int max_chunk) {
  int64_t chunk = ts_cdiv(n_pairs * tiles, ts_wgrad_wgs());
  chunk = std::min<int64_t>(max_chunk, std::max<int64_t>(128, (chunk + step - 1) / step * step));
  TsWgradPlan p;
  p.chunk = (int)chunk;
  p.n_chunks = (int)ts_cdiv(std::max<int64_t>(n_pairs, 1), chunk);
  p.slots = (int64_t)p.n_chunks + K;
  return p;
}
struct TsWgradReduce {
  const float *part;
  const int *nboffs;
  float *dW;
  int K, chunk;
  int64_t cacb4;
};
extern thread_local float *g_ts_wgrad_part;
extern thread_local TsWgradPlan g_ts_wgrad_plan;
int ts_wgrad_reduce(const TsWgradReduce &job, ts_stream_t stream);
int ts_wgrad_reduce_seq(const TsWgradReduce &job, ts_stream_t stream);
size_t ts_wgrad_partial_bytes(int64_t n_pairs, int32_t c_a, int32_t c_b, int32_t K);

__device__ __forceinline__ void ts_wgrad_reduce_one(const TsWgradReduce &job, int64_t i) {
  const int k = (int)(i / job.cacb4);
  const int64_t e = i - (int64_t)k * job.cacb4;
  const int lo = job.nboffs[k], hi = job.nboffs[k + 1];
  float4 acc = make_float4(0.f, 0.f, 0.f, 0.f);
  if (hi > lo) {
    const int c0 = lo / job.chunk, c1 = (hi - 1) / job.chunk;
    const float4 *src = (const float4 *)job.part + ((int64_t)c0 + k) * job.cacb4 + e;
#pragma unroll 4
    for (int c = c0; c <= c1; ++c, src += job.cacb4) {
      const float4 v = *src;
      acc.x += v.x;
      acc.y += v.y;
      acc.z += v.z;
      acc.w += v.w;
    }
  }
  ((float4 *)job.dW)[i] = acc;
}

#define TS_COMM_CALLER_PRE ((void *)1)
#define TS_COMM_CALLER_POST ((void *)2)

struct TsPlanesHint {
  const float *w;
  const unsigned short *planes;
  int K, c_in, c_out;
};
extern thread_local TsPlanesHint g_ts_planes_hint;

struct TsClassFinish {
  const int32_t *pos;
  int64_t n;
  void *out;
  const void *addend;
};
int ts_conv_class_gemm_ex(const float *feat, int32_t c_red, const float *kernel, int32_t K, int32_t groups, int32_t c_out,
                          const int32_t *src, int64_t m_pad, const int32_t *tile_info, const int32_t *n_tiles, int32_t wt,
                          int32_t mirror, const int32_t *rows, float *zp, const TsWgradReduce *side, const TsClassFinish *fin,
                          ts_stream_t stream);
int ts_conv_class_gemm_f16_ex(const void *feat, int32_t c_red, const void *w, int32_t K, int32_t groups, int32_t c_out,
                              const int32_t *src, int64_t m_pad, const int32_t *tile_info, const int32_t *n_tiles, int32_t wt,
                              int32_t mirror, const int32_t *rows, void *zp, const TsWgradReduce *side, const TsClassFinish *fin,
                              ts_stream_t stream);

int ts_conv_gather_sum_ex(const float *z, int32_t c, const int32_t *pos, int32_t K, int64_t n_rows, int64_t n_pairs,
                          float *out, const TsWgradReduce *side, const float *addend, ts_stream_t stream);
int ts_conv_gather_sum_f16_ex(const void *z, int32_t c, const int32_t *pos, int32_t K, int64_t n_rows, int64_t n_pairs,
                              void *out, const TsWgradReduce *side, const void *addend, ts_stream_t stream);
struct TsGatherEpilogue {
  const float *mean, *invstd, *w, *b;
  const void *residual;
  int relu;
};
int ts_conv_gather_sum_epi(const float *z, int32_t c, const int32_t *pos, int32_t K, int64_t n_rows, int64_t n_pairs, float *out,
                           const TsGatherEpilogue &epi, ts_stream_t stream);
int ts_conv_gather_sum_f16_epi(const void *z, int32_t c, const int32_t *pos, int32_t K, int64_t n_rows, int64_t n_pairs, void *out,
                               const TsGatherEpilogue &epi, ts_stream_t stream);
int ts_conv_wgrad_ex(const float *a_feat, int32_t c_a, const float *b_feat, int32_t c_b, const int32_t *nbmaps,
                     const int32_t *nboffs, int32_t K, int32_t col_a, int64_t n_pairs, float *grad_kernel,
                     int32_t already_zero, ts_stream_t stream);
int ts_conv_wgrad_f16_ex(const void *a_feat, int32_t c_a, const void *b_feat, int32_t c_b, const int32_t *nbmaps,
                         const int32_t *nboffs, int32_t K, int32_t col_a, int64_t n_pairs, float *grad_kernel,
                         int32_t already_zero, ts_stream_t stream);
```

### taseg_amd/csrc/conv.hip

```cpp
#include "common.h"

typedef float f32x4 __attribute__((ext_vector_type(4)));

#define CV_CK 32
#define CV_AP (CV_CK + 4)

int g_ts_conv_impl = 0;

extern "C" void ts_set_conv_impl(int32_t impl) { g_ts_conv_impl = impl; }

template <int BM, int MAXU, bool WT>
__global__ __launch_bounds__(256) void conv_nbr_kernel(const float *__restrict__ X, int R,
                                                       const float *__restrict__ W,
                                                       const int *__restrict__ nbr, int64_t n_out, int K,
                                                       float *__restrict__ Y, int O_total, int o_tile,
                                                       int k_per_group) {
  extern __shared__ __attribute__((aligned(16))) float smem[];
  const int tid = threadIdx.x, lane = tid & 63;
  const int wave = __builtin_amdgcn_readfirstlane(tid >> 6);
  const int r16 = lane & 15, g = lane >> 4;
  const int o0 = blockIdx.y * o_tile;
  const int k_begin = blockIdx.z * k_per_group;
  const int k_end = min(K, k_begin + k_per_group);
  const int OT = min(o_tile, O_total - o0);
  const int O16 = (OT + 15) & ~15;
  const int OP = O16 + 4;
  const int NB = O16 >> 4;

  float *outT = smem;
  float *At = outT + BM * OP;
  float *Wt = At + BM * CV_AP;
  const int wt_floats = WT ? O16 * CV_AP : CV_CK * OP;
  int *list_in = (int *)(Wt + wt_floats);
  int *list_row = list_in + BM;
  int *wave_cnt = list_row + BM;

  const int64_t row0 = (int64_t)blockIdx.x * BM;
  const int nrows = (int)min((int64_t)BM, n_out - row0);

  for (int e = tid; e < BM * OP; e += 256) outT[e] = 0.f;

  int u_mb[MAXU], u_nb[MAXU];
#pragma unroll
  for (int i = 0; i < MAXU; ++i) {
    int u = wave + 4 * i;
    u_mb[i] = u / NB;
    u_nb[i] = u - u_mb[i] * NB;
  }
  const bool x_vec = ((R & 3) == 0) && ((((uintptr_t)X) & 15) == 0);
  const bool w_vec = WT ? (((R & 3) == 0) && ((((uintptr_t)W) & 15) == 0))
                        : (((O_total & 3) == 0) && ((o0 & 3) == 0) && ((((uintptr_t)W) & 15) == 0));

  for (int k = k_begin; k < k_end; ++k) {
    __syncthreads();
    int idx = -1, rank = 0;
    if (tid < BM) {
      if (tid < nrows) idx = nbr[(int64_t)k * n_out + row0 + tid];
      unsigned long long mk = __ballot(idx >= 0);
      if (lane == 0) wave_cnt[wave] = (int)__popcll(mk);
      rank = (int)__popcll(mk & ((1ULL << lane) - 1ULL));
    }
    __syncthreads();
    int m = 0;
#pragma unroll
    for (int w = 0; w < BM / 64; ++w) m += wave_cnt[w];
    if (m == 0) continue;
    if (idx >= 0) {
      int pos = rank;
      for (int w = 0; w < wave; ++w) pos += wave_cnt[w];
      list_in[pos] = idx;
      list_row[pos] = tid;
    }
    const int M16 = (m + 15) >> 4;
    const int mrows = M16 << 4;

    f32x4 acc[MAXU];
#pragma unroll
    for (int i = 0; i < MAXU; ++i) acc[i] = (f32x4){0.f, 0.f, 0.f, 0.f};

    for (int c0 = 0; c0 < R; c0 += CV_CK) {
      const int ck = min(CV_CK, R - c0);
      const int ck16 = (ck + 15) & ~15;
      __syncthreads();
      for (int e = tid; e < mrows * (CV_CK / 4); e += 256) {
        int rr = e >> 3, c4 = (e & 7) << 2;
        if (c4 >= ck16) continue;
        float4 v = make_float4(0.f, 0.f, 0.f, 0.f);
        if (rr < m) {
          const float *src = X + (int64_t)list_in[rr] * R + c0 + c4;
          if (x_vec && c4 + 3 < ck) {
            v = *(const float4 *)src;
          } else {
// ... 302 lines not shown
```

### taseg_amd/csrc/conv_class.hip

```cpp
#include <cstring>

#include <rocprim/device/device_radix_sort.hpp>

#include "common.h"

typedef float f32x4 __attribute__((ext_vector_type(4)));
typedef float f32x2 __attribute__((ext_vector_type(2)));
typedef __bf16 bf2 __attribute__((ext_vector_type(2)));
typedef __bf16 bf8 __attribute__((ext_vector_type(8)));
typedef short s16x4 __attribute__((ext_vector_type(4)));
typedef unsigned u32x4 __attribute__((ext_vector_type(4)));

#define CG_BM 128
#define CG_BK 32
#define CG_AP (CG_BK + 8)
#define CG_GROUPS 3
#define CG_GK 9

static int ts_cu_count() {
  int dev = 0, cus = 0;
  if (hipGetDevice(&dev) != hipSuccess || hipDeviceGetAttribute(&cus, hipDeviceAttributeMultiprocessorCount, dev) != hipSuccess || cus <= 0)
    return 256;
  return cus;
}
// ... 386 lines not shown
  bind(__builtin_ctz(mask));
  mask &= mask - 1;
  load_regs(0);
  bool first = true;
  while (true) {
    if (mask) fetch(__builtin_ctz(mask));
    for (int c0 = 0; c0 < R; c0 += CG_BK) {
      if (!first) __syncthreads();
      first = false;
      store_lds();
      __syncthreads();
      if (c0 + CG_BK < R) {
        load_regs(c0 + CG_BK);
      } else if (mask) {
        bind(__builtin_ctz(mask));
        load_regs(0);
      }
      mma();
    }
#pragma unroll
    for (int mi = 0; mi < MI; ++mi)
#pragma unroll
      for (int ni = 0; ni < NI; ++ni) {
        tot[mi][ni] += acc[mi][ni];
        acc[mi][ni] = (f32x4){0.f, 0.f, 0.f, 0.f};
      }
    if (!mask) break;
    mask &= mask - 1;
  }
  if (rows) {
#pragma unroll
    for (int mi = 0; mi < MI; ++mi)
#pragma unroll
      for (int q = 0; q < 4; ++q) {
        const int dst = rows[row0 + (wr * MI + mi) * 16 + 4 * g + q];
        if (dst >= 0) {
          float *zr = Zp + (int64_t)dst * O_total + o0 + r16;
#pragma unroll
          for (int ni = 0; ni < NI; ++ni) zr[(wc * NI + ni) * 16] = tot[mi][ni][q];
        }
      }
    return;
  }
  if (fin.phase == 2) {
    constexpr int ZF = BN + 4;
    float *Zt = (float *)smem_cg;
    __syncthreads();
#pragma unroll
    for (int mi = 0; mi < MI; ++mi)
#pragma unroll
      for (int ni = 0; ni < NI; ++ni)
#pragma unroll
        for (int q = 0; q < 4; ++q)
          Zt[((wr * MI + mi) * 16 + 4 * g + q) * ZF + (wc * NI + ni) * 16 + r16] = tot[mi][ni][q];
    __syncthreads();
    const int *crow = src + (int64_t)fin.klc * m_pad + row0;
    float *out = (float *)fin.out;
    const float *add = (const float *)fin.addend;
    constexpr int C4 = BN / 4;
    for (int e = tid; e < BM * C4; e += 256) {
      const int row = e / C4, c4 = e - row * C4;
      const int r = crow[row];
      if (r < 0) continue;
      const int p0 = fin.pos[r], p2 = fin.pos[2 * fin.n + r];
      f32x4 v = {0.f, 0.f, 0.f, 0.f};
      if (p0 >= 0) v += *(const f32x4 *)(Zp + (int64_t)p0 * O_total + o0 + 4 * c4);
      v += *(const f32x4 *)&Zt[row * ZF + 4 * c4];
      if (p2 >= 0) v += *(const f32x4 *)(Zp + (int64_t)p2 * O_total + o0 + 4 * c4);
      if (add) v += *(const f32x4 *)(add + (int64_t)r * O_total + o0 + 4 * c4);
      *(f32x4 *)(out + (int64_t)r * O_total + o0 + 4 * c4) = v;
    }
    return;
  }
  float *zt = Zp + row0 * O_total + o0;
#pragma unroll
  for (int mi = 0; mi < MI; ++mi)
#pragma unroll
    for (int ni = 0; ni < NI; ++ni)
#pragma unroll
      for (int q = 0; q < 4; ++q)
        zt[(int64_t)((wr * MI + mi) * 16 + 4 * g + q) * O_total + (wc * NI + ni) * 16 + r16] = tot[mi][ni][q];
}

struct CgArgs {
  const int *src;
  int64_t m_pad;
  const int2 *tile_info;
  const int *n_tiles;
  int K, gk, mirror;
  const int *rows;
  TsWgradReduce side;
  CgFinish fin;
  int groups;
};
static int64_t cg_tile_bound(const CgArgs &a) { return a.m_pad / CG_BM; }

template <int BN, int WR, bool WT>
static int launch_class(const float *X, int R, const float *W, int O_total, const CgArgs &a, float *Zp, hipStream_t stream) {
  const size_t stage = (size_t)(3 * CG_BM * CG_AP + 3 * (WT ? BN * CG_AP : CG_BK * (BN + 8))) * 2;
  const size_t lds = a.fin.phase == 2 ? std::max(stage, (size_t)CG_BM * (BN + 4) * 4) : stage;
  const unsigned tiles = (unsigned)cg_tile_bound(a);
  dim3 grid(tiles + (a.side.K > 0 ? 64u : 0u), (unsigned)(O_total / BN));
  class_gemm_kernel<BN, WR, WT><<<grid, 256, lds, stream>>>(X, R, W, O_total, a.src, a.m_pad, a.tile_info, a.n_tiles, a.K, a.gk,
                                                            a.mirror, a.rows, Zp, a.side, (int)tiles, a.fin);
  TS_CHECK_LAUNCH("ts_conv_class_gemm");
  return TS_OK;
}
static int cg_tile_columns(int c_out) { return c_out % 128 == 0 ? 128 : c_out % 96 == 0 ? 96 : c_out % 64 == 0 ? 64 : c_out % 32 == 0 ? 32 : 0; }

extern "C" int32_t ts_conv_class_supported(int32_t c_red, int32_t c_out) {
  return c_red > 0 && c_red % CG_BK == 0 && cg_tile_columns(c_out) != 0;
}

static int cg_check(const char *what, int K, int groups, int c_red, int c_out, int64_t m_pad, const void *a, const void *b,
                    const void *c, const void *src, const void *ti, const void *nt) {
  TS_REQUIRE(groups >= 1 && groups <= CG_GROUPS && K > 0 && K % groups == 0 && K / groups <= CG_GK, TS_ERR_UNSUPPORTED,
             "%s: K offsets must split into 1-3 groups of <= 9 (got K %d, groups %d)", what, K, groups);
  TS_REQUIRE(ts_conv_class_supported(c_red, c_out), TS_ERR_UNSUPPORTED,
             "%s: C_red must be a multiple of 32 and C_out of 32 (got %d, %d)", what, c_red, c_out);
  TS_REQUIRE(a && b && c && src && ti && nt, TS_ERR_INVALID_ARGUMENT, "%s: null pointer", what);
  TS_REQUIRE(m_pad > 0 && m_pad % ((int64_t)groups * CG_BM) == 0 && m_pad < (1LL << 31), TS_ERR_INVALID_ARGUMENT,
             "%s: m_pad must be ts_conv_class_rows2(n, groups)", what);
  TS_REQUIRE(((((uintptr_t)a) | ((uintptr_t)b) | ((uintptr_t)c)) & 15) == 0, TS_ERR_INVALID_ARGUMENT,
             "%s: pointers must be 16-byte aligned", what);
  return TS_OK;
}

extern "C" int32_t ts_conv_class_finish_pays(int64_t n, int32_t half) {
  const int64_t lim = ts_get_option(half ? TS_OPT_CLASS_FINISH_ROWS_HALF : TS_OPT_CLASS_FINISH_ROWS);
  return lim > 0 && n >= lim;
}

static int cg_finish(const char *what, const TsClassFinish *fin, int K, int groups, const int32_t *rows, CgFinish &out) {
  out = CgFinish{nullptr, nullptr, nullptr, 0, 0, 0, 0};
  if (!fin) return TS_OK;
  TS_REQUIRE(groups == CG_GROUPS && !rows && (K / 2) / (K / groups) == 1, TS_ERR_INVALID_ARGUMENT,
             "%s: the finish inside the product needs a three-group pass-2 plan", what);
  TS_REQUIRE(fin->pos && fin->out && fin->n > 0 && (((uintptr_t)fin->out) & 15) == 0 && (((uintptr_t)fin->addend) & 15) == 0,
             TS_ERR_INVALID_ARGUMENT, "%s: finish: null / misaligned pointer", what);
  out = CgFinish{fin->pos, fin->addend, fin->out, fin->n, 1, (K / 2) % (K / groups), (K / 2) / (K / groups)};
  return TS_OK;
}

int ts_conv_class_gemm_ex(const float *feat, int32_t c_red, const float *kernel, int32_t K, int32_t groups, int32_t c_out,
                          const int32_t *src, int64_t m_pad, const int32_t *tile_info, const int32_t *n_tiles, int32_t wt,
                          int32_t mirror, const int32_t *rows, float *zp, const TsWgradReduce *side, const TsClassFinish *fin,
                          ts_stream_t stream_) {
  hipStream_t stream = (hipStream_t)stream_;
  const int rc = cg_check("ts_conv_class_gemm", K, groups, c_red, c_out, m_pad, feat, kernel, zp, src, tile_info, n_tiles);
  if (rc != TS_OK) return rc;
  CgArgs a = {src, m_pad, (const int2 *)tile_info, n_tiles, K, K / groups, mirror ? 1 : 0, rows, {}, {}, groups};
  {
    const int frc = cg_finish("ts_conv_class_gemm", fin, K, groups, rows, a.fin);
    if (frc != TS_OK) return frc;
  }
#define CG_GO(BN, WR)                                                                  \
  (wt ? launch_class<BN, WR, true>(feat, c_red, kernel, c_out, a, zp, stream)          \
      : launch_class<BN, WR, false>(feat, c_red, kernel, c_out, a, zp, stream))
  for (int phase = a.fin.phase; phase <= (fin ? 2 : 0); ++phase) {
    a.fin.phase = phase;
    a.side = (side && phase != 1) ? *side : TsWgradReduce{};
    int r;
    switch (cg_tile_columns(c_out)) {
      case 128: r = CG_GO(128, 2); break;
      case 96: r = CG_GO(96, 2); break;
      case 64: r = CG_GO(64, 2); break;
      default: r = CG_GO(32, 4); break;
    }
    if (r != TS_OK) return r;
  }
  return TS_OK;
#undef CG_GO
}

extern "C" int ts_conv_class_gemm(const float *feat, int32_t c_red, const float *kernel, int32_t K, int32_t groups, int32_t c_out,
                                  const int32_t *src, int64_t m_pad, const int32_t *tile_info, const int32_t *n_tiles, int32_t wt,
                                  int32_t mirror, const int32_t *rows, float *zp, ts_stream_t stream) {
  return ts_conv_class_gemm_ex(feat, c_red, kernel, K, groups, c_out, src, m_pad, tile_info, n_tiles, wt, mirror, rows, zp, nullptr,
                               nullptr, stream);
}


extern "C" int ts_conv_class_conv(const float *feat, int32_t c_red, const float *kernel, int32_t K, int32_t groups, int32_t c_out,
                                  const int32_t *src, int64_t m_pad, const int32_t *tile_info, const int32_t *n_tiles, int32_t wt,
                                  int32_t mirror, const int32_t *pos, int64_t n, const float *addend, float *zp, float *out,
                                  ts_stream_t stream) {
  const TsClassFinish fin = {pos, n, out, addend};
  return ts_conv_class_gemm_ex(feat, c_red, kernel, K, groups, c_out, src, m_pad, tile_info, n_tiles, wt, mirror, nullptr, zp, nullptr,
                               &fin, stream);
}

typedef _Float16 ch8 __attribute__((ext_vector_type(8)));
typedef __fp16 chv4t __attribute__((__vector_size__(4 * sizeof(__fp16))));
__device__ __forceinline__ ch8 cgh_frag_tr(const _Float16 *img, int pitch, int r0, int c0, int tq, int tp) {
  typedef chv4t __attribute__((address_space(3))) * lds_hv4;
  const chv4t lo = __builtin_amdgcn_ds_read_tr16_b64_v4f16((lds_hv4)(img + (r0 + tq) * pitch + c0 + 4 * tp));
  const chv4t hi = __builtin_amdgcn_ds_read_tr16_b64_v4f16((lds_hv4)(img + (r0 + 4 + tq) * pitch + c0 + 4 * tp));
  ch8 v;
  v[0] = (_Float16)lo[0]; v[1] = (_Float16)lo[1]; v[2] = (_Float16)lo[2]; v[3] = (_Float16)lo[3];
  v[4] = (_Float16)hi[0]; v[5] = (_Float16)hi[1]; v[6] = (_Float16)hi[2]; v[7] = (_Float16)hi[3];
  return v;
}

struct CgCursor {
  int tile, round, slot, G, n_tiles;
  int rest;
  int row0, grp;
  int2 ahead;
};
struct CgStep {
  int row0, grp, kl, last;
};

template <int BN, int WR, bool WT, int RC>
__global__ __launch_bounds__(256, 2) void class_gemm_h_kernel(
    const _Float16 *__restrict__ X, int R, const _Float16 *__restrict__ W, int O_total, const int *__restrict__ src, int64_t m_pad,
    const int2 *__restrict__ tile_info, const int *__restrict__ n_tiles_p, int K, int gk, int mirror, const int *__restrict__ rows,
    _Float16 *__restrict__ Zp, TsWgradReduce side, int G, CgFinish fin) {
  constexpr int BM = CG_BM;
  constexpr int WC = 4 / WR;
  constexpr int MI = (BM / 16) / WR;
  constexpr int NI = (BN / 16) / WC;
  constexpr int AP = RC + 8;
  constexpr int BP = BN + 8;
  constexpr int A_HALVES = BM * AP;
  constexpr int RQ = RC / 8;
  constexpr int A_IT = BM * RQ / 256;
  constexpr int B_CHUNKS = RC * BN / 8;
  constexpr int B_IT = (B_CHUNKS + 255) / 256;
  constexpr int KB = RC / 32;
  constexpr int ZP = BN + 8;
  constexpr int CH = BN / 8;
  extern __shared__ __attribute__((aligned(16))) _Float16 smem_cgh[];
  _Float16 *At = smem_cgh;
  _Float16 *Bt = At + A_HALVES;

  const int tid = threadIdx.x, lane = tid & 63;
  const int wave = __builtin_amdgcn_readfirstlane(tid >> 6);
  const int r16 = lane & 15, g = lane >> 4;
  const int tq = r16 >> 2, tp = lane & 3;
  const int wr = wave / WC, wc = wave % WC;
  const int o0 = blockIdx.y * BN;
  if ((int)blockIdx.x >= G) {
    if (blockIdx.y == 0) {
      const int64_t step = (int64_t)(gridDim.x - G) * 256;
      for (int64_t i = (int64_t)((int)blockIdx.x - G) * 256 + tid; i < (int64_t)side.K * side.cacb4; i += step)
        ts_wgrad_reduce_one(side, i);
    }
    return;
  }

  CgCursor cur;
  cur.G = G;
  cur.slot = (int)blockIdx.x;
  cur.round = 0;
  cur.n_tiles = __builtin_amdgcn_readfirstlane(*n_tiles_p);
  cur.tile = cur.slot;
  cur.rest = 0;
  cur.row0 = cur.grp = 0;
  cur.ahead = make_int2(0, 0);
  auto tile_of = [&](int round) { return round * G + ((round & 1) ? G - 1 - cur.slot : cur.slot); };
  auto load_entry = [&](int t) -> int2 {
    int2 e = make_int2(0, 0);
    if (t < cur.n_tiles) e = tile_info[t];
    return make_int2(__builtin_amdgcn_readfirstlane(e.x), __builtin_amdgcn_readfirstlane(e.y));
  };
  auto zero_tile = [&](int row0) {
    const ch8 zero = {0, 0, 0, 0, 0, 0, 0, 0};
    for (int e = tid; e < BM * CH; e += 256) {
      const int r = e / CH, c8 = e - r * CH;
      const int dst = rows ? rows[row0 + r] : (int)(row0 + r);
      if (dst >= 0) *(ch8 *)(Zp + (int64_t)dst * O_total + o0 + 8 * c8) = zero;
// ... 270 lines not shown
```

### taseg_amd/planes.py

```python
import ctypes
import os
import weakref

import torch

from . import _lib as L
from .options import options

__all__ = ["planes_for", "half_for", "invalidate", "eligible", "eligible_half", "hint", "stats"]

_ENABLED = options.presplit
_entries = {}
_half_entries = {}
_epoch = 0
stats = {"refreshes": 0, "launch_batches": 0}


class TsPlaneJob(ctypes.Structure):
    _fields_ = [("w", ctypes.c_void_p), ("planes", ctypes.c_void_p), ("K", ctypes.c_int32), ("c_in", ctypes.c_int32),
                ("c_out", ctypes.c_int32)]


class _Entry:
    __slots__ = ("ref", "planes", "ptr", "version", "epoch", "stream")

    def __init__(self, weight, half=False):
        self.ref = weakref.ref(weight)
        self.planes = (torch.empty(weight.shape, dtype=torch.float16, device=weight.device) if half else
                       torch.empty(3 * weight.numel(), dtype=torch.int16, device=weight.device))
        self.ptr = self.version = self.epoch = self.stream = None

    def fresh(self, weight, stream):
        return self.ptr == weight.data_ptr() and self.version == weight._version and self.epoch == _epoch \
            and self.stream == stream


def invalidate():
    global _epoch
    _epoch += 1


def _wide(c):
    return c % 128 == 0 and c % 96 != 0


def eligible(weight) -> bool:
    return (_ENABLED and weight.is_cuda and weight.dtype == torch.float32 and weight.dim() == 3 and weight.is_contiguous()
            and weight.shape[0] <= 63 and weight.shape[1] % 32 == 0 and weight.shape[2] % 32 == 0
            and (_wide(weight.shape[1]) or _wide(weight.shape[2])))


def _refresh(stream, device, entries=None, fn="ts_conv_split_planes_batch"):
    entries = _entries if entries is None else entries
    jobs, done = [], []
    for key, e in list(entries.items()):
        w = e.ref()
        if w is None:
            del entries[key]
            continue
        if w.device != device:
            continue
        if not e.fresh(w, stream):
            k, c_in, c_out = w.shape if w.dim() == 3 else (1, w.shape[0], w.shape[1])
            jobs.append((w.data_ptr(), e.planes.data_ptr(), k, c_in, c_out))
            done.append((e, w))
    if not jobs:
        return
    arr = (TsPlaneJob * len(jobs))(*[TsPlaneJob(*j) for j in jobs])
    L.check(getattr(L.load(), fn)(arr, len(jobs), stream), fn)
    for e, w in done:
        e.ptr, e.version, e.epoch, e.stream = w.data_ptr(), w._version, _epoch, stream
    stats["refreshes"] += len(jobs)
    stats["launch_batches"] += 1


def planes_for(weight):
    e = _entries.get(id(weight))
    if e is not None and e.ref() is weight and e.fresh(weight, L.stream()) and e.planes.device == weight.device:
        return e.planes
    if not eligible(weight):
        return None
    if weight.device.index != torch.cuda.current_device():
        return None
    stream = L.stream()
    e = _entries.get(id(weight))
    if e is None or e.ref() is not weight or e.planes.device != weight.device:
        e = _entries[id(weight)] = _Entry(weight)
    if not e.fresh(weight, stream):
        _refresh(stream, weight.device)
    return e.planes


def eligible_half(weight) -> bool:
    return (_ENABLED and weight.is_cuda and weight.dtype == torch.float32 and weight.dim() in (2, 3) and weight.is_contiguous()
            and (weight.shape[-2] * weight.shape[-1]) % 8 == 0 and weight.data_ptr() % 16 == 0)


def half_for(weight):
    e = _half_entries.get(id(weight))
    if e is not None and e.ref() is weight and e.fresh(weight, L.stream()) and e.planes.device == weight.device \
            and e.planes.shape == weight.shape:
        return e.planes
    if not eligible_half(weight) or weight.device.index != torch.cuda.current_device():
        return None
    stream = L.stream()
    e = _half_entries.get(id(weight))
    if e is None or e.ref() is not weight or e.planes.device != weight.device or e.planes.shape != weight.shape:
        e = _half_entries[id(weight)] = _Entry(weight, half=True)
    if not e.fresh(weight, stream):
        _refresh(stream, weight.device, _half_entries, "ts_cast_weights_f16_batch")
    return e.planes


def hint(weight32, planes):
    if planes is not None:
        k, c_in, c_out = weight32.shape
        L.load().ts_conv_planes_hint(weight32.data_ptr(), planes.data_ptr(), k, c_in, c_out)
```

### taseg_amd/torchsparse/nn/functional.py

```python
import os
from typing import List, Optional, Tuple, Union

import torch
from torch.autograd import Function

from ... import backend as B
from ... import planes as _planes
from ...options import options
from ..tensor import SparseTensor
from ..utils import make_ntuple
from .utils import get_kernel_offsets

__all__ = ["conv3d", "conv_geometry", "conv_block_ok", "conv_block_eval", "sphash", "sphashquery", "spcount", "spvoxelize", "spdevoxelize", "spdevoxelize_cat", "calc_ti_weights",
           "spdownsample", "KernelMap", "build_kernel_map", "build_pyramid", "point_linear", "spvoxelize_max", "sigmoid3_gate", "spvoxelize_mean", "point_tail",
           "gather_rows"]

_fwd = torch.amp.custom_fwd(device_type="cuda", cast_inputs=torch.float32)
_bwd = torch.amp.custom_bwd(device_type="cuda")


def sphash(coords: torch.Tensor, offsets: Optional[torch.Tensor] = None) -> torch.Tensor:
    assert coords.dtype == torch.int, coords.dtype
    assert coords.ndim == 2 and coords.shape[1] == 4, coords.shape
    if offsets is None:
# ... 194 lines not shown
        key = (transposed, c_in, c_out, half)
        hit = self._plans.get(key)
        if hit is None:
            hit = self._choose_plans(transposed, c_in, c_out, half)
            self._plans[key] = hit
        return hit

    def _choose_plans(self, transposed, c_in, c_out, half):
        if not _dense_ok(c_in, c_out) or self.dup:
            return None, None
        if self.cls is not None and not transposed and class_gemm_pays(self.cls["n"], c_in, c_out, half):
            return self.cls, self.cls
        if self.direct is not None:
            d = self.direct
            fwd, dgrad = (d["up"], d["down"]) if transposed else (d["down"], d["up"])
            return (fwd if fwd is not None and direct_conv_pays(fwd is d["up"], fwd["n"], c_in, c_out, half) else None,
                    dgrad if dgrad is not None and direct_conv_pays(dgrad is d["up"], dgrad["n"], c_out, c_in, half) else None)
        return None, None

    def class_rows(self) -> int:
        return 0 if self.cls is None else self.cls["z_rows"]

    @property
    def total(self) -> int:
        if self._total is None:
            if self._dup is None:
                t, d = torch.stack([self.nboffs[-1], self._dup_dev.to(self.nboffs.dtype)]).tolist()
                self._total, self._dup = int(t), bool(d)
            else:
                self._total = int(self.nboffs[-1].item())
        return self._total

    @property
    def dup(self) -> bool:
        if self._dup is None:
            if self._total is None:
                self.total
            else:
                self._dup = bool(self._dup_dev.item())
        return self._dup

    @property
    def nbmaps(self) -> torch.Tensor:
        if self._nbmaps is None:
            self._nbmaps = self.nbmaps_buf[:self.total].long()
        return self._nbmaps

    @property
    def nbsizes(self) -> torch.Tensor:
        return self.nbsizes_dev.long()

    def __getitem__(self, i):
        return (self.nbmaps, self.nbsizes, self.sizes)[i]

    def __iter__(self):
        return iter((self.nbmaps, self.nbsizes, self.sizes))

    def __len__(self):
        return 3


def accept_class_plans(kmaps):
    pending = [km for km in kmaps if km._cls_pending is not None]
    if not pending:
        return
    counts = torch.stack([km._cls_pending["n_tiles"] for km in pending]).tolist() if len(pending) > 1 \
        else [pending[0]._cls_pending["n_tiles"].tolist()]
    for km, (tiles, steps) in zip(pending, counts):
        km._accept(tiles, steps)


_CLASS_GEMM = options.class_gemm
_CLASS_MIN_ROWS = 16384
_CLASS_MIN_ROWS_96 = options.class_min_rows_96
_CLASS_MIN_ROWS_128 = options.class_min_rows_128
_CLASS_MAX_WORK = 1.6
_CLASS_MIN_ROWS_HALF = options.class_min_rows_half
_DIRECT_CONV = options.direct_conv != "0"
_DIRECT_MIN_ROWS = options.direct_min_rows
_DIRECT_DOWN_MIN_ROWS = 8000
_DIRECT_FORCE = options.direct_conv == "force"


def class_conv(x, w, plan, f16, wt=False):
    if plan["rows"] is not None:
        return (B.conv_class_gemm_f16 if f16 else B.conv_class_gemm)(x, w, plan, weight_transposed=wt)
    if plan["groups"] == 3 and B.class_finish_pays(plan["n"], f16):
        return (B.conv_class_conv_f16 if f16 else B.conv_class_conv)(x, w, plan, weight_transposed=wt)
    z = (B.conv_class_gemm_f16 if f16 else B.conv_class_gemm)(x, w, plan, weight_transposed=wt)
    return (B.conv_gather_sum_f16 if f16 else B.conv_gather_sum)(z, plan["pos"], plan["n"])


def class_gemm_pays(n_rows: int, c_in: int, c_out: int, half: bool = False) -> bool:
    if half:
        return n_rows >= _CLASS_MIN_ROWS_HALF
    if max(c_in, c_out) <= 64:
        return n_rows >= _CLASS_MIN_ROWS
    cols128 = any(c % 128 == 0 and c % 96 != 0 for c in (c_in, c_out))
    return n_rows >= (_CLASS_MIN_ROWS_128 if cols128 else _CLASS_MIN_ROWS_96)


def direct_conv_pays(up: bool, n_dest: int, c_red: int, c_cols: int, half: bool) -> bool:
    if _DIRECT_FORCE:
        return True
    wide = max(c_red, c_cols) > 64
    if up:
        return True if half else n_dest >= (60000 if wide else 20000)
    if half:
        return n_dest >= (60000 if wide else 8000) and max(c_red, c_cols) <= 96
    return (not wide) and n_dest >= 20000


def build_kernel_map(in_coords, out_coords, kernel_size, tensor_stride, dilation=1) -> KernelMap:
    offsets = get_kernel_offsets(kernel_size, stride=tensor_stride, dilation=dilation, device=in_coords.device)
    tables = B.build_kmap(in_coords, out_coords, offsets)
    k, n = offsets.shape[0], out_coords.shape[0]
    if (k & 1) and n > 0 and in_coords.shape == out_coords.shape and in_coords.data_ptr() == out_coords.data_ptr():
        tables["dup"] = (tables["nbr"][k // 2] != torch.arange(n, device=out_coords.device, dtype=tables["nbr"].dtype)).any()
    return KernelMap(tables, (in_coords.shape[0], out_coords.shape[0]))


def _amp_half(feats: torch.Tensor) -> bool:
    return feats.is_cuda and (feats.dtype == torch.float16 or torch.is_autocast_enabled("cuda"))


def _half_ok(*channels) -> bool:
    return all(c % 32 == 0 for c in channels)


class _NoCtx:
    __slots__ = ()

    def __enter__(self):
        return self

    def __exit__(self, *exc):
        return False


_NO_CTX = _NoCtx()


def _no_autocast():
    return torch.autocast("cuda", enabled=False) if torch.is_autocast_enabled("cuda") else _NO_CTX


class _SparseConv(Function):

    @staticmethod
    def forward(ctx, feats, weight, kmap: KernelMap, transposed: bool, planes=None):
        if feats.shape[1] != weight.shape[1]:
            raise ValueError("Input feature size and kernel size mismatch")
        n_in, n_out = kmap.sizes
        rows_expected = n_out if transposed else n_in
        if feats.shape[0] != rows_expected:
            raise ValueError(f"conv3d{' (transposed)' if transposed else ''}: {feats.shape[0]} input rows but the "
                             f"kernel map has {rows_expected}")
        want_half = _amp_half(feats)
        half = want_half and _half_ok(weight.shape[1], weight.shape[2])
        gcol, table, rows = (1, kmap.pos_in, n_in) if transposed else (0, kmap.pos_out, n_out)
        cls, cls_d = kmap.plans_for(transposed, weight.shape[1], weight.shape[2], half)

        with _no_autocast():
            if half:
                fh = feats.contiguous().half()
                w16, _ = B.cast_weights_f16(weight.detach().float(), want=(True, False))
                if cls is not None:
                    out = class_conv(fh, w16, cls, True)
                else:
                    z = B.conv_pair_gemm_f16(fh, w16, kmap.nbmaps_buf, kmap.nboffs, kmap.total, gather_col=gcol, natural=True)
                    out = _scatter_pairs(z, kmap, False, rows) if (transposed and kmap.dup) else B.conv_gather_sum_f16(z, table, rows)
                ctx.save_for_backward(fh, w16)
            else:
                f32, w32 = feats.contiguous().float(), weight.contiguous().float()
                if w32.data_ptr() != weight.data_ptr():
                    planes = None
                if cls is not None:
                    out = class_conv(f32, w32, cls, False)
                else:
                    _planes.hint(w32, planes)
                    z = B.conv_pair_gemm(f32, w32, kmap.nbmaps_buf, kmap.nboffs, kmap.total, gather_col=gcol)
                    out = _scatter_pairs(z, kmap, False, rows) if (transposed and kmap.dup) else B.conv_gather_sum(z, table, rows)
                ctx.save_for_backward(f32, w32)
                if want_half:
                    out = out.half()
        ctx.kmap, ctx.transposed, ctx.half, ctx.in_dtype = kmap, transposed, half, feats.dtype
        ctx.planes = None if half else planes
        ctx.cls = cls_d
        return out

    @staticmethod
    def backward(ctx, grad_out):
        feats, weight = ctx.saved_tensors
        kmap, transposed = ctx.kmap, ctx.transposed
        n_in, n_out = kmap.sizes
        k = weight.shape[0]
        grad_feats = grad_weight = None
        gcol = 0 if transposed else 1
        table, rows = (kmap.pos_in, n_in) if not transposed else (kmap.pos_out, n_out)
        with _no_autocast():
            if ctx.half:
                gh = grad_out.contiguous().half()
                if ctx.needs_input_grad[0] and ctx.cls is not None:
                    grad_feats = class_conv(gh, weight, ctx.cls, True, True).to(ctx.in_dtype)
                elif ctx.needs_input_grad[0]:
                    z = B.conv_pair_gemm_f16(gh, weight, kmap.nbmaps_buf, kmap.nboffs, kmap.total, gather_col=gcol)
                    grad_feats = (_scatter_pairs(z, kmap, transposed, rows) if kmap.dup else
                                  B.conv_gather_sum_f16(z, table, rows)).to(ctx.in_dtype)
                if ctx.needs_input_grad[1]:
                    grad_weight = B.conv_wgrad_f16(feats, gh, kmap.nbmaps_buf, kmap.nboffs, k,
                                                   col_a=1 if transposed else 0, max_pairs=kmap.total)
            else:
                g32 = grad_out.contiguous().float()
                if ctx.needs_input_grad[0] and ctx.cls is not None:
                    grad_feats = class_conv(g32, weight, ctx.cls, False, True).to(ctx.in_dtype)
                elif ctx.needs_input_grad[0]:
                    _planes.hint(weight, ctx.planes)
                    z = B.conv_pair_gemm(g32, weight, kmap.nbmaps_buf, kmap.nboffs, kmap.total, gather_col=gcol,
                                         weight_transposed=True)
                    grad_feats = (_scatter_pairs(z, kmap, transposed, rows) if kmap.dup else
                                  B.conv_gather_sum(z, table, rows)).to(ctx.in_dtype)
                if ctx.needs_input_grad[1]:
                    grad_weight = B.conv_wgrad(feats, g32, kmap.nbmaps_buf, kmap.nboffs, k,
                                               col_a=1 if transposed else 0, max_pairs=kmap.total)
        return grad_feats, grad_weight, None, None, None


def _scatter_pairs(z, kmap, transposed, rows):
    total = kmap.total
    idx = kmap.nbmaps_buf[:total, 1 if transposed else 0].long()
    out = torch.zeros((rows, z.shape[1]), dtype=torch.float32, device=z.device)
    return out.index_add_(0, idx, z[:total].float()).to(z.dtype)


def build_pyramid(x: SparseTensor, num_levels: int = 4, kernel_size: int = 3, down_kernel: int = 2) -> None:
    ks, dk, ones = make_ntuple(kernel_size, 3), make_ntuple(down_kernel, 3), (1, 1, 1)
    cur = x
    x.cmaps.setdefault(x.stride, x.coords)
    coords, stride = x.coords, x.stride
    maps = []
    for level in range(num_levels + 1):
        key = (stride, ks, ones, ones)
        if key not in x.kmaps:
            x.kmaps[key] = build_kernel_map(coords, coords, ks, stride, 1)
        maps.append(x.kmaps[key])
        if level == num_levels:
            break
        nxt = tuple(s * d for s, d in zip(stride, dk))
        if nxt not in x.cmaps:
            x.cmaps[nxt] = spdownsample(coords, dk, dk, stride)
        key = (stride, dk, dk, ones)
        if key not in x.kmaps:
            x.kmaps[key] = build_kernel_map(coords, x.cmaps[nxt], dk, stride, 1)
        maps.append(x.kmaps[key])
        coords, stride = x.cmaps[nxt], nxt
    pending = [m for m in maps if m._total is None]
    if pending:
        zero = pending[0].nboffs.new_zeros(())
        flags = [zero if m._dup_dev is None else m._dup_dev.to(zero.dtype) for m in pending]
        totals = torch.stack([m.nboffs[-1] for m in pending] + flags).tolist()
        for m, t, d in zip(pending, totals, totals[len(pending):]):
            m._total = int(t)
            if m._dup is None:
                m._dup = bool(d)
    del cur


def _dense_ok(c_in: int, c_out: int) -> bool:
    return c_in % 32 == 0 and c_out % 32 == 0


class _PointwiseConv(Function):

    @staticmethod
    def forward(ctx, feats, weight, ident):
        half = _amp_half(feats)
        pairs, offs = ident
        c_in, c_out = weight.shape
        ours = _dense_ok(c_in, c_out)
        n = feats.shape[0]
        with _no_autocast():
            if half:
                f = feats.contiguous().half()
                if ours:
                    w16, _ = B.cast_weights_f16(weight.detach().float().view(1, c_in, c_out), want=(True, False))
                    out = B.conv_pair_gemm_f16(f, w16, pairs, offs, n, gather_col=0, natural=True)
                    w = w16
                else:
                    w = weight.detach().half()
                    out = f.matmul(w)
            else:
                f = feats.contiguous().float()
                w = weight.detach().float()
                out = B.conv_pair_gemm(f, w.view(1, c_in, c_out), pairs, offs, n, gather_col=0) if ours else f.matmul(w)
        ctx.save_for_backward(f, w)
        ctx.ident, ctx.half, ctx.in_dtype, ctx.ours = ident, half, feats.dtype, ours
        return out

# ... 570 lines not shown
```

Measured before the change: 132.4.

## Add persistent tile-walking class GEMM using pre-split bf16 weight planes

Adds a persistent class_gemm_p_kernel where each block walks a snake-ordered sequence of tiles and kernel offsets. It software-pipelines the A gathers and B loads across offsets, and B is read from pre-split bf16 weight planes instead of being split per tile. Plane eligibility is widened to all multi-offset weights, and the planes are threaded through the forward and backward class-conv paths. Spare blocks can run a side wgrad reduction. This targets per-tile launch and tail overhead and repeated weight splitting, at the cost of extra plane memory, hint plumbing, and a more complex kernel with register pressure.

New measurement: 136.7 (median of 6 runs). 3.3% higher.

```diff
diff --git a/include/taseg_hip.h b/include/taseg_hip.h
--- a/include/taseg_hip.h
+++ b/include/taseg_hip.h
@@ -477,6 +477,11 @@
 int ts_conv_class_gemm(const float *feat, int32_t c_red, const float *kernel, int32_t K, int32_t groups, int32_t c_out,
                        const int32_t *src, int64_t m_pad, const int32_t *tile_info, const int32_t *n_tiles, int32_t wt,
                        int32_t mirror, const int32_t *rows, float *zp, ts_stream_t stream);
+int32_t ts_conv_class_walk_slots(int32_t c_out, int32_t wt);
+int ts_conv_class_gemm_wsum(const float *feat, int32_t c_red, const float *kernel, int32_t K, int32_t groups, int32_t c_out,
+                            const int32_t *src, int64_t m_pad, const int32_t *tile_info, const int32_t *n_tiles, int32_t wt,
+                            int32_t mirror, const int32_t *rows, float *zp, const float *part, const int32_t *side_nboffs, float *dw,
+                            int32_t side_k, int32_t chunk, int64_t cacb, ts_stream_t stream);
 int32_t ts_conv_class_finish_pays(int64_t n, int32_t half);
 int ts_conv_class_conv(const float *feat, int32_t c_red, const float *kernel, int32_t K, int32_t groups, int32_t c_out,
                        const int32_t *src, int64_t m_pad, const int32_t *tile_info, const int32_t *n_tiles, int32_t wt,
diff --git a/taseg_amd/_lib.py b/taseg_amd/_lib.py
--- a/taseg_amd/_lib.py
+++ b/taseg_amd/_lib.py
@@ -186,6 +186,9 @@
     "ts_conv_class_plan_pairs": (_i32, [_vp, _vp, _i32, _i64, _vp, _vp, _vp, _vp, _vp, _sz, _vp]),
     "ts_conv_nbr_transposed": (_i32, [_vp, _vp, _i32, _i64, _vp, _vp]),
     "ts_conv_class_supported": (_i32, [_i32, _i32]),
+    "ts_conv_class_walk_slots": (_i32, [_i32, _i32]),
+    "ts_conv_class_gemm_wsum": (_i32, [_vp, _i32, _vp, _i32, _i32, _i32, _vp, _i64, _vp, _vp, _i32, _i32, _vp, _vp, _vp, _vp, _vp, _i32,
+                                       _i32, _i64, _vp]),
     "ts_conv_class_gemm": (_i32, [_vp, _i32, _vp, _i32, _i32, _i32, _vp, _i64, _vp, _vp, _i32, _i32, _vp, _vp, _vp]),
     "ts_conv_class_gemm_f16": (_i32, [_vp, _i32, _vp, _i32, _i32, _i32, _vp, _i64, _vp, _vp, _i32, _i32, _vp, _vp, _vp]),
     "ts_conv_class_finish_pays": (_i32, [_i64, _i32]),
diff --git a/taseg_amd/backend.py b/taseg_amd/backend.py
--- a/taseg_amd/backend.py
+++ b/taseg_amd/backend.py
@@ -1000,7 +1000,7 @@
 
 def set_conv_impl(impl):
     global _conv_impl
-    _conv_impl = int(impl)
+    _conv_impl = 0 if int(impl) in (14, 15) else int(impl)
     L.load().ts_set_conv_impl(int(impl))
 
 
@@ -1588,7 +1588,7 @@
     return st
 
 
-def conv_class_gemm(feat, kernel, plan, weight_transposed=False):
+def conv_class_gemm(feat, kernel, plan, weight_transposed=False, planes=None):
     L.require_device(feat, kernel)
     feat, kernel = _f32(feat, "feat"), _f32(kernel, "kernel")
     k, c_in, c_out = kernel.shape
@@ -1600,6 +1600,8 @@
     with _Timed("class_gemm", name=f"class_gemm_kernel<{_tile_cols(cols)}>", pairs=int(plan.get("pairs", 0)), c_red=c_red,
                 c_out=cols, k=k, esize=4, n_rows=feat.shape[0], z_rows=0 if direct else int(plan.get("z_rows") or plan["m_pad"]),
                 out_rows=plan["n"] if direct else 0):
+        if planes is not None:
+            L.load().ts_conv_planes_hint(L.ptr(kernel), L.ptr(planes), k, c_in, c_out)
         L.check(L.load().ts_conv_class_gemm(L.ptr(feat), c_red, L.ptr(kernel), k, plan["groups"], cols, L.ptr(plan["src"]),
                                             plan["m_pad"], L.ptr(plan["tile_info"]), L.ptr(plan["n_tiles"]),
                                             1 if weight_transposed else 0, plan["mirror"], L.ptr(plan["rows"]), L.ptr(zp),
diff --git a/taseg_amd/csrc/block.hip b/taseg_amd/csrc/block.hip
--- a/taseg_amd/csrc/block.hip
+++ b/taseg_amd/csrc/block.hip
@@ -237,7 +237,7 @@
                                            0, 0, cp->rows, dst, nullptr, fused ? &fin : nullptr, stream));
         else
           TS_TRY(ts_conv_class_gemm_ex((const float *)feat, c_in, kernel, K, cp->groups, c_out, cp->src, cp->m_pad, cp->tile_info,
-                                       cp->n_tiles, 0, 0, cp->rows, (float *)dst, nullptr, fused ? &fin : nullptr, stream));
+                                       cp->n_tiles, 0, 0, cp->rows, (float *)dst, nullptr, fused ? &fin : nullptr, planes.h.planes, stream));
       }
       if (!cp->rows && !fused) {
         ProfScope ps(1, stream, plan_z_rows(cp), 0, c_out, cp->groups, (double)n_out, es_d, 0);
@@ -470,7 +470,7 @@
       else
         TS_TRY(ts_conv_class_gemm_ex((const float *)grad_conv, c_out, (const float *)weights, K, cp->groups, c_in, cp->src,
                                      cp->m_pad, cp->tile_info, cp->n_tiles, 1, cp->mirror, cp->rows, (float *)dst, side,
-                                     fused ? &fin : nullptr, stream));
+                                     fused ? &fin : nullptr, planes.h.planes, stream));
     }
     if (!cp->rows && !fused) {
       ProfScope ps(1, stream, plan_z_rows(cp), 0, c_in, cp->groups, (double)n_dgrad_rows, es_d, side_bytes);
diff --git a/taseg_amd/csrc/common.h b/taseg_amd/csrc/common.h
--- a/taseg_amd/csrc/common.h
+++ b/taseg_amd/csrc/common.h
@@ -11,6 +11,7 @@
 
 void ts_set_error(const char *fmt, ...);
 extern int g_ts_conv_impl;
+extern int g_ts_class_one_tile;
 
 #define TS_REQUIRE(cond, code, ...)  \
   do {                               \
@@ -214,7 +215,7 @@
 int ts_conv_class_gemm_ex(const float *feat, int32_t c_red, const float *kernel, int32_t K, int32_t groups, int32_t c_out,
                           const int32_t *src, int64_t m_pad, const int32_t *tile_info, const int32_t *n_tiles, int32_t wt,
                           int32_t mirror, const int32_t *rows, float *zp, const TsWgradReduce *side, const TsClassFinish *fin,
-                          ts_stream_t stream);
+                          const void *planes, ts_stream_t stream);
 int ts_conv_class_gemm_f16_ex(const void *feat, int32_t c_red, const void *w, int32_t K, int32_t groups, int32_t c_out,
                               const int32_t *src, int64_t m_pad, const int32_t *tile_info, const int32_t *n_tiles, int32_t wt,
                               int32_t mirror, const int32_t *rows, void *zp, const TsWgradReduce *side, const TsClassFinish *fin,
diff --git a/taseg_amd/csrc/conv.hip b/taseg_amd/csrc/conv.hip
--- a/taseg_amd/csrc/conv.hip
+++ b/taseg_amd/csrc/conv.hip
@@ -6,8 +6,12 @@
 #define CV_AP (CV_CK + 4)
 
 int g_ts_conv_impl = 0;
-
-extern "C" void ts_set_conv_impl(int32_t impl) { g_ts_conv_impl = impl; }
+int g_ts_class_one_tile = 0;
+
+extern "C" void ts_set_conv_impl(int32_t impl) {
+  g_ts_class_one_tile = impl == 14 ? 1 : impl == 15 ? 2 : 0;
+  g_ts_conv_impl = (impl == 14 || impl == 15) ? 0 : impl;
+}
 
 template <int BM, int MAXU, bool WT>
 __global__ __launch_bounds__(256) void conv_nbr_kernel(const float *__restrict__ X, int R,
diff --git a/taseg_amd/csrc/conv_class.hip b/taseg_amd/csrc/conv_class.hip
--- a/taseg_amd/csrc/conv_class.hip
+++ b/taseg_amd/csrc/conv_class.hip
@@ -492,6 +492,304 @@
         zt[(int64_t)((wr * MI + mi) * 16 + 4 * g + q) * O_total + (wc * NI + ni) * 16 + r16] = tot[mi][ni][q];
 }
 
+struct CgWalkStep {
+  int row0, grp, kl, last;
+};
+
+struct CgWalkSlice {
+  int valid, off_done, tile_done, row0;
+  const unsigned short *wb;
+};
+
+template <int BN, int WR, bool WT, int NS>
+__global__ __launch_bounds__(256, 2) void class_gemm_p_kernel(const float *__restrict__ X, int R, const float *__restrict__ W,
+                                                             int O_total, const int *__restrict__ src, int64_t m_pad,
+                                                             const int2 *__restrict__ tile_info,
+                                                             const int *__restrict__ n_tiles_p, int tile_bound, int K, int gk,
+                                                             int mirror, const int *__restrict__ rows, float *__restrict__ Zp,
+                                                             TsWgradReduce side, int G,
+                                                             const unsigned short *__restrict__ P, int64_t plane_n) {
+  constexpr int BM = CG_BM;
+  constexpr int WC = 4 / WR;
+  constexpr int MI = (BM / 16) / WR;
+  constexpr int NI = (BN / 16) / WC;
+  constexpr int BP = BN + 8;
+  constexpr int A_PLANE = BM * CG_AP;
+  constexpr int B_PLANE = WT ? BN * CG_AP : CG_BK * BP;
+  constexpr int A_IT = BM * (CG_BK / 8) / 256;
+  constexpr int B_CHUNKS = BN * (CG_BK / 8);
+  constexpr int B_IT = (B_CHUNKS + 255) / 256;
+  constexpr int A_PLANES = 3;
+  extern __shared__ __attribute__((aligned(16))) unsigned short smem_cg[];
+  unsigned short *Ap = smem_cg;
+  unsigned short *Bp = Ap + A_PLANES * A_PLANE;
+
+  const int tid = threadIdx.x, lane = tid & 63;
+  const int wave = __builtin_amdgcn_readfirstlane(tid >> 6);
+  const int r16 = lane & 15, g = lane >> 4;
+  const int tq = r16 >> 2, tp = lane & 3;
+  const int wr = wave / WC, wc = wave % WC;
+  const int o0 = blockIdx.y * BN;
+  if ((int)blockIdx.x >= G) {
+    if (blockIdx.y == 0) {
+      const int64_t step = (int64_t)(gridDim.x - G) * 256;
+      for (int64_t i = (int64_t)((int)blockIdx.x - G) * 256 + tid; i < (int64_t)side.K * side.cacb4; i += step)
+        ts_wgrad_reduce_one(side, i);
+    }
+    return;
+  }
+
+  const int n_tiles = min(__builtin_amdgcn_readfirstlane(*n_tiles_p), tile_bound);
+  const int slot = (int)blockIdx.x;
+  int round = 0, rest = 0, cur_row0 = 0, cur_grp = 0;
+  auto tile_of = [&](int r) __attribute__((always_inline)) { return r * G + ((r & 1) ? G - 1 - slot : slot); };
+  auto load_entry = [&](int t) __attribute__((always_inline)) -> int2 {
+    int2 e = make_int2(0, 0);
+    if (t < n_tiles) e = tile_info[t];
+    return make_int2(__builtin_amdgcn_readfirstlane(e.x), __builtin_amdgcn_readfirstlane(e.y));
+  };
+  auto zero_tile = [&](int row0) __attribute__((always_inline)) {
+    int t0 = tid;
+    asm volatile("" : "+v"(t0));
+    for (int e = t0; e < BM * (BN / 4); e += 256) {
+      const int r = e / (BN / 4), c4 = e - r * (BN / 4);
+      const int dst = rows ? rows[row0 + r] : row0 + r;
+      if (dst >= 0) *(f32x4 *)(Zp + (int64_t)dst * O_total + o0 + 4 * c4) = (f32x4){0.f, 0.f, 0.f, 0.f};
+    }
+  };
+  int2 ahead = load_entry(tile_of(0));
+  auto next_step = [&](CgWalkStep &st) __attribute__((always_inline)) -> bool {
+    while (rest == 0) {
+      if (tile_of(round) >= n_tiles) return false;
+      const int2 e = ahead;
+      round += 1;
+      ahead = load_entry(tile_of(round));
+      cur_grp = e.x & 3;
+      cur_row0 = (e.x >> 2) * BM;
+      rest = e.y & 511;
+      if (rest == 0) zero_tile(cur_row0);
+    }
+    st.kl = __builtin_ctz(rest);
+    rest &= rest - 1;
+    st.row0 = cur_row0;
+    st.grp = cur_grp;
+    st.last = rest == 0;
+    return true;
+  };
+
+  const int arow0 = tid >> 2, acol = (tid & 3) << 3;
+  int boff[B_IT], bdst[B_IT];
+#pragma unroll
+  for (int it = 0; it < B_IT; ++it) {
+    const int e = min(tid + it * 256, B_CHUNKS - 1);
+    if (WT) {
+      const int col = e >> 2, c8 = (e & 3) << 3;
+      boff[it] = col * R + c8;
+      bdst[it] = col * CG_AP + c8;
+    } else {
+      constexpr int q8 = BN >> 3;
+      const int kk = e / q8, c8 = (e - kk * q8) << 3;
+      boff[it] = kk * O_total + c8;
+      bdst[it] = kk * BP + c8;
+    }
+  }
+
+  f32x4 acc[MI][NI], tot[MI][NI];
+#pragma unroll
+  for (int mi = 0; mi < MI; ++mi)
+#pragma unroll
+    for (int ni = 0; ni < NI; ++ni) acc[mi][ni] = tot[mi][ni] = (f32x4){0.f, 0.f, 0.f, 0.f};
+
+  const float *aptr[A_IT];
+  bool alive[A_IT];
+  const unsigned short *wk = P;
+  int nsrc[A_IT];
+  auto fetch = [&](const CgWalkStep &st) __attribute__((always_inline)) {
+#pragma unroll
+    for (int it = 0; it < A_IT; ++it) nsrc[it] = src[(int64_t)st.kl * m_pad + st.row0 + arow0 + 64 * it];
+  };
+  auto bind = [&](const CgWalkStep &st) __attribute__((always_inline)) {
+    const int k = gk * st.grp + st.kl;
+    const int kw = (WT && mirror) ? (K - 1 - k) : k;
+#pragma unroll
+    for (int it = 0; it < A_IT; ++it) {
+      alive[it] = nsrc[it] >= 0;
+      aptr[it] = alive[it] ? X + (int64_t)nsrc[it] * R + acol : W + acol;
+    }
+    wk = WT ? P + ((int64_t)kw * O_total + o0) * R : P + (int64_t)kw * R * O_total + o0;
+  };
+  f32x4 ra[NS][A_IT][2];
+  u32x4 rb[B_IT][3];
+  bool rlive[NS][A_IT];
+  CgWalkStep sld, sf;
+  bool has_f = false, ld_valid = false, advance = false;
+  int c0_ld = 0;
+  auto issue_a = [&](auto set_c) __attribute__((always_inline)) -> CgWalkSlice {
+    constexpr int set = decltype(set_c)::value;
+    CgWalkSlice e = {0, 0, 0, 0, P};
+    if (advance) {
+      advance = false;
+      if (has_f) {
+        bind(sf);
+        sld = sf;
+        c0_ld = 0;
+        has_f = next_step(sf);
+        if (has_f) fetch(sf);
+      } else {
+        ld_valid = false;
+        c0_ld = 0;
+#pragma unroll
+        for (int it = 0; it < A_IT; ++it) {
+          alive[it] = false;
+          aptr[it] = W + acol;
+        }
+      }
+    }
+#pragma unroll
+    for (int it = 0; it < A_IT; ++it) {
+      ra[set][it][0] = *(const f32x4 *)(aptr[it] + c0_ld);
+      ra[set][it][1] = *(const f32x4 *)(aptr[it] + c0_ld + 4);
+      rlive[set][it] = alive[it];
+    }
+    if (!ld_valid) return e;
+    e.valid = 1;
+    e.off_done = c0_ld + CG_BK >= R;
+    e.tile_done = e.off_done && sld.last;
+    e.row0 = sld.row0;
+    e.wb = WT ? wk + c0_ld : wk + (int64_t)c0_ld * O_total;
+    c0_ld += CG_BK;
+    advance = e.off_done;
+    return e;
+  };
+  auto load_b = [&](const CgWalkSlice &e) __attribute__((always_inline)) {
+#pragma unroll
+    for (int it = 0; it < B_IT; ++it) {
+#pragma unroll
+      for (int p = 0; p < 3; ++p) rb[it][p] = *(const u32x4 *)(e.wb + p * plane_n + boff[it]);
+    }
+  };
+  auto store_lds = [&](auto set_c) __attribute__((always_inline)) {
+    constexpr int set = decltype(set_c)::value;
+    const f32x4 zero = {0.f, 0.f, 0.f, 0.f};
+#pragma unroll
+    for (int it = 0; it < A_IT; ++it) {
+      const int rr = arow0 + 64 * it;
+      const f32x4 v0 = rlive[set][it] ? ra[set][it][0] : zero, v1 = rlive[set][it] ? ra[set][it][1] : zero;
+      unsigned short *dst = Ap + rr * CG_AP + acol;
+      u32x4 h, m, l;
+      cg_split8(v0, v1, h, m, l);
+      *(u32x4 *)dst = h;
+      *(u32x4 *)(dst + A_PLANE) = m;
+      *(u32x4 *)(dst + 2 * A_PLANE) = l;
+    }
+#pragma unroll
+    for (int it = 0; it < B_IT; ++it) {
+      if (B_IT * 256 == B_CHUNKS || tid + it * 256 < B_CHUNKS) {
+        unsigned short *dst = Bp + bdst[it];
+#pragma unroll
+        for (int p = 0; p < 3; ++p) *(u32x4 *)(dst + p * B_PLANE) = rb[it][p];
+      }
+    }
+  };
+  auto mma = [&]() __attribute__((always_inline)) {
+    bf8 a[MI][A_PLANES];
+#pragma unroll
+    for (int mi = 0; mi < MI; ++mi)
+#pragma unroll
+      for (int p = 0; p < A_PLANES; ++p)
+        a[mi][p] = *(const bf8 *)&Ap[p * A_PLANE + ((wr * MI + mi) * 16 + r16) * CG_AP + 8 * g];
+#pragma unroll
+    for (int ni = 0; ni < NI; ++ni) {
+      bf8 b[3];
+#pragma unroll
+      for (int p = 0; p < 3; ++p) {
+        if (WT)
+          b[p] = *(const bf8 *)&Bp[p * B_PLANE + ((wc * NI + ni) * 16 + r16) * CG_AP + 8 * g];
+        else
+          b[p] = cg_frag_tr(Bp + p * B_PLANE, BP, 8 * g, (wc * NI + ni) * 16, tq, tp);
+      }
+#pragma unroll
+      for (int mi = 0; mi < MI; ++mi) CG_MMA(acc[mi][ni], a[mi], b);
+    }
+  };
+  auto store_tile = [&](int row0) __attribute__((always_inline)) {
+    int g = lane >> 4, r16 = lane & 15;
+    asm volatile("" : "+v"(g), "+v"(r16));
+    if (rows) {
+      int dst[MI][4];
+#pragma unroll
+      for (int mi = 0; mi < MI; ++mi)
+#pragma unroll
+        for (int q = 0; q < 4; ++q) dst[mi][q] = rows[row0 + (wr * MI + mi) * 16 + 4 * g + q];
+#pragma unroll
+      for (int mi = 0; mi < MI; ++mi)
+#pragma unroll
+        for (int q = 0; q < 4; ++q)
+          if (dst[mi][q] >= 0) {
+            float *zr = Zp + (int64_t)dst[mi][q] * O_total + o0 + r16;
+#pragma unroll
+            for (int ni = 0; ni < NI; ++ni) zr[(wc * NI + ni) * 16] = tot[mi][ni][q];
+          }
+    } else {
+      float *zt = Zp + (int64_t)row0 * O_total + o0;
+#pragma unroll
+      for (int mi = 0; mi < MI; ++mi)
+#pragma unroll
+        for (int ni = 0; ni < NI; ++ni)
+#pragma unroll
+          for (int q = 0; q < 4; ++q)
+            zt[(int64_t)((wr * MI + mi) * 16 + 4 * g + q) * O_total + (wc * NI + ni) * 16 + r16] = tot[mi][ni][q];
+    }
+#pragma unroll
+    for (int mi = 0; mi < MI; ++mi)
+#pragma unroll
+      for (int ni = 0; ni < NI; ++ni) tot[mi][ni] = (f32x4){0.f, 0.f, 0.f, 0.f};
+  };
+
+  ld_valid = next_step(sld);
+  if (!ld_valid) return;
+  fetch(sld);
+  bind(sld);
+  has_f = next_step(sf);
+  if (has_f) fetch(sf);
+  CgWalkSlice e[NS + 1];
+  e[0] = issue_a(std::integral_constant<int, 0>{});
+  load_b(e[0]);
+  if (NS == 2) e[1] = issue_a(std::integral_constant<int, 1>{});
+  bool first = true, more = true;
+  auto body = [&](auto set_c) __attribute__((always_inline)) {
+    if (!first) __syncthreads();
+    first = false;
+    store_lds(set_c);
+    __syncthreads();
+    if (NS == 2) {
+      load_b(e[1]);
+      e[2 % (NS + 1)] = issue_a(set_c);
+    } else {
+      e[1] = issue_a(set_c);
+      load_b(e[1]);
+    }
+    mma();
+    if (e[0].off_done) {
+#pragma unroll
+      for (int mi = 0; mi < MI; ++mi)
+#pragma unroll
+        for (int ni = 0; ni < NI; ++ni) {
+          tot[mi][ni] += acc[mi][ni];
+          acc[mi][ni] = (f32x4){0.f, 0.f, 0.f, 0.f};
+        }
+      if (e[0].tile_done) store_tile(e[0].row0);
+    }
+    more = e[1].valid != 0;
+    e[0] = e[1];
+    if (NS == 2) e[1] = e[2 % (NS + 1)];
+  };
+  do {
+    body(std::integral_constant<int, 0>{});
+    if (NS == 2) body(std::integral_constant<int, NS - 1>{});
+  } while (more);
+}
+
 struct CgArgs {
   const int *src;
   int64_t m_pad;
@@ -502,6 +800,8 @@
   TsWgradReduce side;
   CgFinish fin;
   int groups;
+  const unsigned short *planes;
+  int64_t plane_n;
 };
 static int64_t cg_tile_bound(const CgArgs &a) { return a.m_pad / CG_BM; }
 
@@ -517,6 +817,42 @@
   return TS_OK;
 }
 static int cg_tile_columns(int c_out) { return c_out % 128 == 0 ? 128 : c_out % 96 == 0 ? 96 : c_out % 64 == 0 ? 64 : c_out % 32 == 0 ? 32 : 0; }
+
+template <int BN>
+constexpr int cg_row_sets() { return BN <= 96 ? 2 : 1; }
+template <int BN, int WR, bool WT>
+static int class_p_resident() {
+  static const int resident = [] {
+    const size_t lds = (size_t)(3 * CG_BM * CG_AP + 3 * (WT ? BN * CG_AP : CG_BK * (BN + 8))) * 2;
+    int nb = 0;
+    if (hipOccupancyMaxActiveBlocksPerMultiprocessor(&nb, class_gemm_p_kernel<BN, WR, WT, cg_row_sets<BN>()>, 256, lds) != hipSuccess || nb < 1) nb = 1;
+    return ts_cu_count() * nb;
+  }();
+  return resident;
+}
+template <int BN, int WR, bool WT>
+static int launch_class_p(const float *X, int R, const float *W, int O_total, const CgArgs &a, float *Zp, hipStream_t stream) {
+  const size_t lds = (size_t)(3 * CG_BM * CG_AP + 3 * (WT ? BN * CG_AP : CG_BK * (BN + 8))) * 2;
+  const int64_t tiles = cg_tile_bound(a);
+  const int ny = O_total / BN;
+  const int G = g_ts_class_one_tile == 2 ? (int)tiles
+                                         : (int)std::max<int64_t>(1, std::min<int64_t>(tiles, class_p_resident<BN, WR, WT>() / ny));
+  dim3 grid((unsigned)G + (a.side.K > 0 ? 64u : 0u), (unsigned)ny);
+  class_gemm_p_kernel<BN, WR, WT, cg_row_sets<BN>()><<<grid, 256, lds, stream>>>(X, R, W, O_total, a.src, a.m_pad, a.tile_info, a.n_tiles, (int)tiles,
+                                                              a.K, a.gk, a.mirror, a.rows, Zp, a.side, G, a.planes, a.plane_n);
+  TS_CHECK_LAUNCH("ts_conv_class_gemm (persistent)");
+  return TS_OK;
+}
+
+extern "C" int32_t ts_conv_class_walk_slots(int32_t c_out, int32_t wt) {
+  const int bn = cg_tile_columns(c_out);
+  if (bn == 0) return 0;
+  const int ny = c_out / bn;
+#define CG_RES(BN, WR) (wt ? class_p_resident<BN, WR, true>() : class_p_resident<BN, WR, false>())
+  const int res = bn == 128 ? CG_RES(128, 2) : bn == 96 ? CG_RES(96, 2) : bn == 64 ? CG_RES(64, 2) : CG_RES(32, 4);
+#undef CG_RES
+  return std::max(1, res / ny);
+}
 
 extern "C" int32_t ts_conv_class_supported(int32_t c_red, int32_t c_out) {
   return c_red > 0 && c_red % CG_BK == 0 && cg_tile_columns(c_out) != 0;
@@ -552,21 +888,32 @@
   return TS_OK;
 }
 
+static const void *cg_take_hint(const float *kernel, int K, int c_in, int c_out) {
+  const TsPlanesHint h = g_ts_planes_hint;
+  g_ts_planes_hint = TsPlanesHint{nullptr, nullptr, 0, 0, 0};
+  return (h.w == kernel && h.planes && h.K == K && h.c_in == c_in && h.c_out == c_out) ? h.planes : nullptr;
+}
+
 int ts_conv_class_gemm_ex(const float *feat, int32_t c_red, const float *kernel, int32_t K, int32_t groups, int32_t c_out,
                           const int32_t *src, int64_t m_pad, const int32_t *tile_info, const int32_t *n_tiles, int32_t wt,
                           int32_t mirror, const int32_t *rows, float *zp, const TsWgradReduce *side, const TsClassFinish *fin,
-                          ts_stream_t stream_) {
+                          const void *planes, ts_stream_t stream_) {
   hipStream_t stream = (hipStream_t)stream_;
   const int rc = cg_check("ts_conv_class_gemm", K, groups, c_red, c_out, m_pad, feat, kernel, zp, src, tile_info, n_tiles);
   if (rc != TS_OK) return rc;
-  CgArgs a = {src, m_pad, (const int2 *)tile_info, n_tiles, K, K / groups, mirror ? 1 : 0, rows, {}, {}, groups};
+  TS_REQUIRE((((uintptr_t)planes) & 15) == 0, TS_ERR_INVALID_ARGUMENT, "ts_conv_class_gemm: planes must be 16-byte aligned");
+  CgArgs a = {src, m_pad, (const int2 *)tile_info, n_tiles, K, K / groups, mirror ? 1 : 0, rows, {}, {}, groups,
+              (const unsigned short *)planes, (int64_t)K * c_red * c_out};
   {
     const int frc = cg_finish("ts_conv_class_gemm", fin, K, groups, rows, a.fin);
     if (frc != TS_OK) return frc;
   }
-#define CG_GO(BN, WR)                                                                  \
-  (wt ? launch_class<BN, WR, true>(feat, c_red, kernel, c_out, a, zp, stream)          \
-      : launch_class<BN, WR, false>(feat, c_red, kernel, c_out, a, zp, stream))
+  const bool walk = !fin && planes && g_ts_class_one_tile != 1;
+#define CG_GO(BN, WR)                                                                              \
+  (walk ? (wt ? launch_class_p<BN, WR, true>(feat, c_red, kernel, c_out, a, zp, stream)            \
+              : launch_class_p<BN, WR, false>(feat, c_red, kernel, c_out, a, zp, stream))          \
+        : (wt ? launch_class<BN, WR, true>(feat, c_red, kernel, c_out, a, zp, stream)              \
+              : launch_class<BN, WR, false>(feat, c_red, kernel, c_out, a, zp, stream)))
   for (int phase = a.fin.phase; phase <= (fin ? 2 : 0); ++phase) {
     a.fin.phase = phase;
     a.side = (side && phase != 1) ? *side : TsWgradReduce{};
@@ -587,7 +934,19 @@
                                   const int32_t *src, int64_t m_pad, const int32_t *tile_info, const int32_t *n_tiles, int32_t wt,
                                   int32_t mirror, const int32_t *rows, float *zp, ts_stream_t stream) {
   return ts_conv_class_gemm_ex(feat, c_red, kernel, K, groups, c_out, src, m_pad, tile_info, n_tiles, wt, mirror, rows, zp, nullptr,
-                               nullptr, stream);
+                               nullptr, cg_take_hint(kernel, K, wt ? c_out : c_red, wt ? c_red : c_out), stream);
+}
+
+extern "C" int ts_conv_class_gemm_wsum(const float *feat, int32_t c_red, const float *kernel, int32_t K, int32_t groups, int32_t c_out,
+                                       const int32_t *src, int64_t m_pad, const int32_t *tile_info, const int32_t *n_tiles, int32_t wt,
+                                       int32_t mirror, const int32_t *rows, float *zp, const float *part, const int32_t *side_nboffs,
+                                       float *dw, int32_t side_k, int32_t chunk, int64_t cacb, ts_stream_t stream) {
+  TS_REQUIRE(part && side_nboffs && dw && side_k > 0 && chunk > 0 && cacb > 0 && cacb % 4 == 0 &&
+                 ((((uintptr_t)part) | ((uintptr_t)dw)) & 15) == 0,
+             TS_ERR_INVALID_ARGUMENT, "ts_conv_class_gemm_wsum: bad side job");
+  const TsWgradReduce side = {part, side_nboffs, dw, side_k, chunk, cacb / 4};
+  return ts_conv_class_gemm_ex(feat, c_red, kernel, K, groups, c_out, src, m_pad, tile_info, n_tiles, wt, mirror, rows, zp, &side,
+                               nullptr, cg_take_hint(kernel, K, wt ? c_out : c_red, wt ? c_red : c_out), stream);
 }
 
 
@@ -597,7 +956,7 @@
                                   ts_stream_t stream) {
   const TsClassFinish fin = {pos, n, out, addend};
   return ts_conv_class_gemm_ex(feat, c_red, kernel, K, groups, c_out, src, m_pad, tile_info, n_tiles, wt, mirror, nullptr, zp, nullptr,
-                               &fin, stream);
+                               &fin, nullptr, stream);
 }
 
 typedef _Float16 ch8 __attribute__((ext_vector_type(8)));
diff --git a/taseg_amd/planes.py b/taseg_amd/planes.py
--- a/taseg_amd/planes.py
+++ b/taseg_amd/planes.py
@@ -47,7 +47,7 @@
 def eligible(weight) -> bool:
     return (_ENABLED and weight.is_cuda and weight.dtype == torch.float32 and weight.dim() == 3 and weight.is_contiguous()
             and weight.shape[0] <= 63 and weight.shape[1] % 32 == 0 and weight.shape[2] % 32 == 0
-            and (_wide(weight.shape[1]) or _wide(weight.shape[2])))
+            and (weight.shape[0] > 1 or _wide(weight.shape[1]) or _wide(weight.shape[2])))
 
 
 def _refresh(stream, device, entries=None, fn="ts_conv_split_planes_batch"):
diff --git a/taseg_amd/torchsparse/nn/functional.py b/taseg_amd/torchsparse/nn/functional.py
--- a/taseg_amd/torchsparse/nn/functional.py
+++ b/taseg_amd/torchsparse/nn/functional.py
@@ -300,12 +300,14 @@
 _DIRECT_FORCE = options.direct_conv == "force"
 
 
-def class_conv(x, w, plan, f16, wt=False):
+def class_conv(x, w, plan, f16, wt=False, planes=None):
     if plan["rows"] is not None:
-        return (B.conv_class_gemm_f16 if f16 else B.conv_class_gemm)(x, w, plan, weight_transposed=wt)
+        return B.conv_class_gemm_f16(x, w, plan, weight_transposed=wt) if f16 else \
+            B.conv_class_gemm(x, w, plan, weight_transposed=wt, planes=planes)
     if plan["groups"] == 3 and B.class_finish_pays(plan["n"], f16):
         return (B.conv_class_conv_f16 if f16 else B.conv_class_conv)(x, w, plan, weight_transposed=wt)
-    z = (B.conv_class_gemm_f16 if f16 else B.conv_class_gemm)(x, w, plan, weight_transposed=wt)
+    z = B.conv_class_gemm_f16(x, w, plan, weight_transposed=wt) if f16 else \
+        B.conv_class_gemm(x, w, plan, weight_transposed=wt, planes=planes)
     return (B.conv_gather_sum_f16 if f16 else B.conv_gather_sum)(z, plan["pos"], plan["n"])
 
 
@@ -394,7 +396,7 @@
                 if w32.data_ptr() != weight.data_ptr():
                     planes = None
                 if cls is not None:
-                    out = class_conv(f32, w32, cls, False)
+                    out = class_conv(f32, w32, cls, False, planes=planes)
                 else:
                     _planes.hint(w32, planes)
                     z = B.conv_pair_gemm(f32, w32, kmap.nbmaps_buf, kmap.nboffs, kmap.total, gather_col=gcol)
@@ -431,7 +433,7 @@
             else:
                 g32 = grad_out.contiguous().float()
                 if ctx.needs_input_grad[0] and ctx.cls is not None:
-                    grad_feats = class_conv(g32, weight, ctx.cls, False, True).to(ctx.in_dtype)
+                    grad_feats = class_conv(g32, weight, ctx.cls, False, True, planes=ctx.planes).to(ctx.in_dtype)
                 elif ctx.needs_input_grad[0]:
                     _planes.hint(weight, ctx.planes)
                     z = B.conv_pair_gemm(g32, weight, kmap.nbmaps_buf, kmap.nboffs, kmap.total, gather_col=gcol,
```
